# SamArgt/AudioSourceSep

Hardware: AMD Instinct MI355X
Metric: Glow fwd+logdet passes/sec on 64×64×1 mel tiles (K=32,L=3), 1→8 MI355X (higher is better)
Workload: dtype f16x3

## Files before the change

### audiosourcesep_amd/_lib.py

```python
import ctypes
import os

_HERE = os.path.dirname(os.path.abspath(__file__))
LIB_PATH = os.environ.get("GLOWK_LIB") or os.path.join(_HERE, "libglowk.so")


class GlowkLibraryMissing(RuntimeError):
    pass


class GlowkError(RuntimeError):
    pass


class GlowkRangeError(GlowkError):
    """GLOWK_ERR_RANGE: a call in a split arithmetic (f16x3 / f16x2) left the fp16 range; its outputs are not usable."""


class GlowkConfigStruct(ctypes.Structure):
    _fields_ = [
        ("H", ctypes.c_int32), ("W", ctypes.c_int32), ("C", ctypes.c_int32),
        ("L", ctypes.c_int32), ("K", ctypes.c_int32), ("F", ctypes.c_int32),
        ("learntop", ctypes.c_int32), ("use_logit", ctypes.c_int32),
        ("minval", ctypes.c_float), ("maxval", ctypes.c_float), ("alpha", ctypes.c_float),
        ("bn_eps", ctypes.c_float),
    ]


class GlowkProfile(ctypes.Structure):
    _fields_ = [("net_ms", ctypes.c_double * 4), ("net_launches", ctypes.c_int64 * 4)]


STEP_TENSOR_IDS = {
    "actnorm/log_scale": 0, "actnorm/shift": 1,
    "inv1x1/P": 2, "inv1x1/sign_S": 3, "inv1x1/L": 4, "inv1x1/log_S": 5, "inv1x1/U": 6,
    "nn/conv1/kernel": 7, "nn/conv1/bias": 8,
    "nn/bn1/gamma": 9, "nn/bn1/beta": 10, "nn/bn1/mean": 11, "nn/bn1/var": 12,
    "nn/conv2/kernel": 13, "nn/conv2/bias": 14,
    "nn/bn2/gamma": 15, "nn/bn2/beta": 16, "nn/bn2/mean": 17, "nn/bn2/var": 18,
    "nn/conv3/kernel": 19, "nn/conv3/bias": 20,
    "inv1x1/P_inv": 21,
}
PRIOR_TENSOR_IDS = {"prior/loc": 100, "prior/log_scale": 101}
PREC_F32, PREC_F16X3, PREC_F16X2 = 0, 1, 2
OK, ERR, ERR_RANGE = 0, 1, 2
RANGE_IGNORE, RANGE_ERROR, RANGE_FALLBACK = 0, 1, 2
MIX_DB, MIX_MEAN = 0, 1

_vp, _i, _fp = ctypes.c_void_p, ctypes.c_int, ctypes.POINTER(ctypes.c_float)

SYMBOLS = {
    "glowk_version": (_i, []),
    "glowk_last_error": (ctypes.c_char_p, []),
    "glowk_reload_env": (None, []),
    "glowk_create": (_i, [ctypes.POINTER(GlowkConfigStruct), _i, ctypes.POINTER(_vp)]),
    "glowk_destroy": (_i, [_vp]),
    "glowk_tensor_size": (ctypes.c_size_t, [_vp, _i, _i]),
    "glowk_set_tensor": (_i, [_vp, _i, _i, _i, _fp, ctypes.c_size_t]),
    "glowk_get_tensor": (_i, [_vp, _i, _i, _i, _fp, ctypes.c_size_t]),
    "glowk_finalize_weights": (_i, [_vp]),
    "glowk_actnorm_data_init": (_i, [_vp, _vp, _i, _i, _i, _vp]),
    "glowk_set_precision": (_i, [_vp, _i]),
    "glowk_get_precision": (_i, [_vp]),
    "glowk_set_range_policy": (_i, [_vp, _i]),
    "glowk_get_range_policy": (_i, [_vp]),
    "glowk_range_status": (_i, [_vp, ctypes.POINTER(_i), ctypes.POINTER(ctypes.c_int64), _vp]),
    "glowk_range_probe_begin": (_i, [_vp]),
    "glowk_range_probe_end": (_i, [_vp, ctypes.POINTER(ctypes.c_float), ctypes.POINTER(ctypes.c_float), _vp]),
    "glowk_workspace_bytes": (ctypes.c_size_t, [_vp, _i, _i]),
    "glowk_reserve": (_i, [_vp, _i, _i]),
    "glowk_max_tiles": (_i, [_vp]),
    "glowk_forward": (_i, [_vp, _vp, _i, _vp, _vp, _vp]),
    "glowk_inverse": (_i, [_vp, _vp, _i, _vp, _vp]),
    "glowk_log_prob": (_i, [_vp, _vp, _i, _vp, _vp, _vp]),
    "glowk_log_prob_sum": (_i, [_vp, _vp, _i, _vp, _vp, _vp, _i, _vp]),
    "glowk_sum_f64": (_i, [_vp, ctypes.c_size_t, _vp, _i, ctypes.c_double, _vp]),
    "glowk_log_prob_grad": (_i, [_vp, _vp, _i, _vp, _vp, _vp]),
    "glowk_sample": (_i, [_vp, _vp, _i, _vp, _vp]),
    "glowk_prior_log_prob": (_i, [_vp, _vp, _i, _vp, _vp]),
    "glowk_fused_steps": (ctypes.c_int64, [_vp]),
    "glowk_kernel_families": (_i, [_vp, ctypes.POINTER(ctypes.c_int64)]),
    "glowk_profile_begin": (_i, [_vp]),
    "glowk_profile_end": (_i, [_vp, ctypes.POINTER(GlowkProfile)]),
    "glowk_squeeze": (_i, [_vp, _i, _i, _i, _i, _vp, _vp]),
    "glowk_unsqueeze": (_i, [_vp, _i, _i, _i, _i, _vp, _vp]),
    "glowk_preprocess_forward": (_i, [_vp, _vp, _i, _vp, _vp, _vp]),
    "glowk_preprocess_inverse": (_i, [_vp, _vp, _i, _vp, _vp]),
    "glowk_step_forward": (_i, [_vp, _i, _i, _vp, _i, _vp, _vp, _vp]),
    "glowk_step_inverse": (_i, [_vp, _i, _i, _vp, _i, _vp, _vp]),
    "glowk_coupling_net": (_i, [_vp, _i, _i, _vp, _i, _vp, _vp, _vp]),
    "glowk_param_vector_size": (ctypes.c_size_t, [_vp]),
    "glowk_param_offset": (_i, [_vp, _i, _i, _i, ctypes.POINTER(ctypes.c_size_t), ctypes.POINTER(ctypes.c_size_t)]),
    "glowk_param_grad": (_i, [_vp, _vp, _i, ctypes.c_float, _vp, _vp, _vp]),
    "glowk_apply_gradients": (_i, [_vp, _vp, _i, ctypes.c_float, _vp]),
    "glowk_crc32c": (ctypes.c_uint32, [_vp, ctypes.c_size_t]),
    "glowk_basis_update": (_i, [_vp, _vp, _vp, _vp, _vp, ctypes.c_size_t, ctypes.c_float, ctypes.c_float, _vp, _vp,
                                ctypes.c_uint64, ctypes.c_uint64, ctypes.c_uint64, _vp, _vp]),
    "glowk_basis_mix": (_i, [_vp, _vp, _vp, ctypes.c_size_t, _vp]),
    "glowk_basis_update_n": (_i, [_vp, _vp, _vp, _i, _vp, ctypes.c_size_t, _i, ctypes.c_float, ctypes.c_float,
                                  ctypes.c_uint64, ctypes.c_uint64, ctypes.c_uint64, _vp, _vp]),
    "glowk_basis_mix_n": (_i, [_vp, _i, _vp, ctypes.c_size_t, _i, _vp]),
    "glowk_random_source": (_i, [_vp, ctypes.c_size_t, ctypes.c_uint64, ctypes.c_uint64, _i, _i, _i, ctypes.c_uint64, _vp]),
    "glowk_random": (_i, [_vp, ctypes.c_size_t, ctypes.c_uint64, ctypes.c_uint64, _i, _i, ctypes.c_uint64, _vp]),
    "glowk_add_noise": (_i, [_vp, _vp, ctypes.c_size_t, ctypes.c_float, ctypes.c_uint64, ctypes.c_uint64, _i, ctypes.c_uint64, _vp]),
    "glowk_mel_filterbank": (_i, [_fp]),
    "glowk_mel_frontend": (_i, [_vp, _i, _i, ctypes.c_float, _vp, _vp, _vp]),
    "glowk_mel_to_power": (_i, [_vp, _i, _i, _i, _vp, _vp]),
    "glowk_masked_istft": (_i, [_vp, _i, _vp, _i, _i, _i, _vp, _vp]),
    "glowk_griffinlim": (_i, [_vp, _vp, _i, _i, _i, ctypes.c_float, _vp, _vp]),
    "glowk_resample_length": (ctypes.c_int64, [ctypes.c_int64, _i, _i]),
    "glowk_resample_filter": (_i, [ctypes.POINTER(ctypes.c_double)]),
    "glowk_resample": (_i, [_vp, _i, ctypes.c_int64, _i, _i, _vp, _vp]),
    "glowk_bss_xcorr":(_i, [_vp, _i, ctypes.c_int64, _vp, _i, ctypes.c_int64, _vp, _i, _i, _vp, _vp]),
    "glowk_bss_solve": (_i, [_vp, _i, _i, _i, _i, _i, _vp, _i, _vp, _vp, _vp]),
    "glowk_bss_project": (_i, [_vp, ctypes.c_int64, _i, _i, _i, _vp, _i, ctypes.c_int64, _vp, _i, _vp, _i, _vp, _vp]),
    "glowk_sp_stft": (_i, [_vp, _i, ctypes.c_int64, _vp, _vp]),
    "glowk_sp_istft": (_i, [_vp, _i, _i, ctypes.c_int64, _vp, _vp]),
    "glowk_oracle_mask": (_i, [_vp, _i, _i, _i, _i, ctypes.c_double, ctypes.c_double, _vp, _vp]),
    "glowk_mwf": (_i, [_vp, _i, _i, _vp]),
    "glowk_oracle_mel": (_i, [_vp, _vp, _i, ctypes.c_int64, _i, _i, ctypes.c_double, _vp, _vp]),
    "glowk_mwf_em": (_i, [_vp, _vp, _i, _i, _i, _i, _vp, _vp, _vp]),
    "glowk_mel_frames": (_i, [_vp, _i, ctypes.c_int64, _vp, _vp, _vp]),
    "glowk_tile_cut": (_i, [_vp, _i, _i, _i, _i, ctypes.c_float, _vp, _vp]),
    "glowk_tile_stitch": (_i, [_vp, _i, _i, _i, _i, _i, _vp, _vp]),
}

_lib = None


def load():
    global _lib
    if _lib is not None:
        return _lib
    if not os.path.exists(LIB_PATH):
        raise GlowkLibraryMissing(
            "HIP library %s not found: build it first (python -c 'import __graft_entry__ as g; g.build()'). "
            "There is no CPU fallback for the compute path." % LIB_PATH)
    import torch
    lib = ctypes.CDLL(LIB_PATH)
    for name, (res, args) in SYMBOLS.items():
        fn = getattr(lib, name)
        fn.restype = res
        fn.argtypes = args
    _lib = lib
    return lib


def check(rc):
    if rc != 0:
        msg = load().glowk_last_error()
        raise (GlowkRangeError if rc == ERR_RANGE else GlowkError)(msg.decode() if msg else "glowk error %d" % rc)
```

### audiosourcesep_amd/csrc/glowk.hip

```cpp
#include "glowk_engine.h"
#include "glowk_light.h"

namespace glowk_eng {
thread_local std::string g_err;
}
using namespace glowk_eng;

namespace glowk_eng {

}

namespace glowk_detail {
int num_cus() {
  static int n = 0;
  if (n == 0) {
    int dev = 0; hipDeviceProp_t prop;
    if (hipGetDevice(&dev) == hipSuccess && hipGetDeviceProperties(&prop, dev) == hipSuccess) n = prop.multiProcessorCount;
    if (n <= 0) n = 256;
  }
  return n;
}
void launch_fail(const std::string& m) { fail(m); }
static EnvSwitches read_env() {
  auto on = [](const char* n) { return getenv(n) != nullptr; };
  return EnvSwitches{on("GLOWK_BWD_LIGHT_4"), on("GLOWK_NO_FUSE"), on("GLOWK_WGRAD_PLAIN"), on("GLOWK_CO_OFF"), on("GLOWK_CO_RING3"), on("GLOWK_Q_OFF"), on("GLOWK_CO_TRAIN_OFF"),
                     on("GLOWK_TRAIN_RECOMPUTE"), on("GLOWK_TRAIN_PERSTEP"), on("GLOWK_NO_PRESUM"), on("GLOWK_PG_JOIN")};
}
static EnvSwitches g_env = read_env();
const EnvSwitches& env() { return g_env; }
void reload_env() { g_env = read_env(); }
#define GLOWK_EXTERN_NET(CI_, NF_) extern template NetLaunch launch_net_t<CI_, NF_>(const NetArgs&, NetCall, hipStream_t, bool);
GLOWK_NET_SHAPES(GLOWK_EXTERN_NET)
#undef GLOWK_EXTERN_NET
}

namespace glowk_eng {
using glowk_detail::num_cus;
using glowk_detail::launch_net_t;

NetCall net_call(const glowk_handle* h, int dir, bool store, bool split) {
  if (h->precision == GLOWK_PREC_F32 || !split) return NetCall{dir, NET_EXACT, store};
  return NetCall{dir, h->precision == GLOWK_PREC_F16X2 && dir == NET_FWD && !store ? NET_SPLIT2 : NET_SPLIT3, store};
}

int* flagp(const glowk_handle* h) { return h->precision == GLOWK_PREC_F32 ? nullptr : h->d_flag; }

float bwd_norm_target(float xlim_b) {
  if (!(xlim_b >= 0.125f)) return 0.0f;
  int e = 0;
  std::frexp(xlim_b * 0.5f, &e);
  return std::ldexp(1.0f, std::min(e - 1, 10));
}

NetLaunch launch_net_raw(int c, int F, const NetArgs& a, NetCall call, hipStream_t s, bool dry) {
#define NETCASE(CI_, NF_) if (c == 2 * CI_ && F == 32 * NF_) return launch_net_t<CI_, NF_>(a, call, s, dry);
  GLOWK_NET_SHAPES(NETCASE)
#undef NETCASE
  return glowk_detail::net_failed("unsupported (channels, n_filters) combination: c=" + std::to_string(c) + " F=" + std::to_string(F));
}

int launch_net(glowk_handle* h, int level, int c, int F, const NetArgs& a, hipStream_t s, NetCall call, NetLaunch* out = nullptr) {
  if (h->profiling) {
    while (h->ev_pool.size() < h->ev_used + 2) {
      OwnedEvent e;
      HIPCHK(event_create(e, hipEventDefault));
      h->ev_pool.push_back(std::move(e));
    }
    HIPCHK(hipEventRecord(h->ev_pool[h->ev_used], s));
  }
  const NetLaunch r = launch_net_raw(c, F, a, call, s);
  if (!r.failed) {
    ++h->family_launches[r.family];
    if (r.co) ++h->family_launches[FAM_CO];
    if (r.q) ++h->family_launches[FAM_Q];
  }
  if (h->profiling) {
    HIPCHK(hipEventRecord(h->ev_pool[h->ev_used + 1], s));
    h->ev_used += 2;
    h->ev_level.push_back(level);
  }
  if (out) *out = r;
  return r.failed ? 1 : 0;
}


int launch_bwd_light(int c, const BwdArgs& a, int N, hipStream_t s) {
  const bool wide = c >= 8 && (a.Q + 15) / 16 <= 8 * num_cus() && !glowk_detail::env().bwd_light_4;
  auto al16 = [](const void* p) { return (reinterpret_cast<uintptr_t>(p) & 15) == 0; };
  const bool one = (a.Q + 255) / 256 >= 2 * num_cus() && al16(a.ghalf_in) && al16(a.v) && al16(a.osave) && al16(a.g_o) && al16(a.ghalf_out) &&
                   al16(a.gu_out) && al16(a.gv_out) && !glowk_detail::env().bwd_light_4;
  if (one) { CDISPATCH(c, hipLaunchKernelGGL((k_bwd_light<CC, 1>), dim3((a.Q + 255) / 256), dim3(256), 0, s, a)); }
  else if (wide) { CDISPATCH(c, hipLaunchKernelGGL((k_bwd_light<CC, 16>), dim3((a.Q + 15) / 16), dim3(256), 0, s, a)); }
  else { CDISPATCH(c, hipLaunchKernelGGL((k_bwd_light<CC, 4>), dim3((a.Q + 63) / 64), dim3(256), 0, s, a)); }
  LAUNCHCHK("k_bwd_light");
  return 0;
}

struct FlatLd { double* slot; int stride, base; };

#define PDISPATCH(c, CALL)                                                                     \
  switch (c) {                                                                                 \
    case 8: { constexpr int CC = 8; CALL; } break;                                             \
    case 16: { constexpr int CC = 16; CALL; } break;                                           \
    default: return fail("pre-summed P at channel count " + std::to_string(c));                \
  }

int launch_couple(int c, const CoupleArgs& a, int N, hipStream_t s, const FlatLd* fl = nullptr, bool* flat_used = nullptr) {
  const int hw = a.h * a.w;
  if (N < 2 * num_cus() && hw % 64 == 0 && (!a.logdet || (fl && fl->slot))) {
    CoupleArgs b = a;
    b.logdet = nullptr;
    double* slots = a.logdet ? fl->slot : (double*)nullptr;
    const bool wide = c >= 8 && (a.Q + 15) / 16 <= 8 * num_cus();
    if (a.presum) {
      if (wide) { PDISPATCH(c, hipLaunchKernelGGL((k_couple_flat<CC, 16, true>), dim3((a.Q + 15) / 16), dim3(256), 0, s, b, slots, fl ? fl->stride : 0, fl ? fl->base : 0)); }
      else { PDISPATCH(c, hipLaunchKernelGGL((k_couple_flat<CC, 4, true>), dim3((a.Q + 63) / 64), dim3(256), 0, s, b, slots, fl ? fl->stride : 0, fl ? fl->base : 0)); }
    }
    else if (wide) { CDISPATCH(c, hipLaunchKernelGGL((k_couple_flat<CC, 16>), dim3((a.Q + 15) / 16), dim3(256), 0, s, b, slots, fl ? fl->stride : 0, fl ? fl->base : 0)); }
    else { CDISPATCH(c, hipLaunchKernelGGL((k_couple_flat<CC, 4>), dim3((a.Q + 63) / 64), dim3(256), 0, s, b, slots, fl ? fl->stride : 0, fl ? fl->base : 0)); }
    LAUNCHCHK("k_couple_flat");
    if (flat_used && a.logdet) *flat_used = true;
    return 0;
  }
  if (N >= 2 * num_cus()) {
    if (a.presum) { PDISPATCH(c, hipLaunchKernelGGL((k_couple<CC, false, true>), dim3(N), dim3(256), 0, s, a)); }
    else { CDISPATCH(c, hipLaunchKernelGGL((k_couple<CC, false>), dim3(N), dim3(256), 0, s, a)); }
  } else {
    const int threads = hw >= 256 ? 1024 : hw > 64 ? 512 : 256;
    if (a.presum) { PDISPATCH(c, hipLaunchKernelGGL((k_couple<CC, true, true>), dim3(N), dim3(threads), 0, s, a)); }
    else { CDISPATCH(c, hipLaunchKernelGGL((k_couple<CC, true>), dim3(N), dim3(threads), 0, s, a)); }
  }
  LAUNCHCHK("k_couple");
  return 0;
}

bool fuse_geometry_ok(int h, int w, int pxw = 256) {
  const int hw = h * w;
  if (w < 4 || w > FUSE_EW || (w & (w - 1)) || pxw % w) return false;
  if (hw % pxw == 0) return true;
  return hw >= 32 && hw < pxw && (hw & (hw - 1)) == 0;
}

int net_and_couple(glowk_handle* h, int lvl, int c, int F, NetArgs na, CoupleArgs ca, int N, hipStream_t s, NetCall call, const FlatLd* fl = nullptr,
                   bool* flat_used = nullptr) {
  const bool no_fuse = glowk_detail::env().no_fuse;
  const bool fusable = call.arith != NET_EXACT && call.dir != NET_BWD && !call.store;
  const int hw = ca.h * ca.w;
  if (!no_fuse && c == 4 && fusable && na.RSp && ca.vin && !ca.log_s_out && ca.out && na.in_stride == 4 &&
      ca.out_stride % 4 == 0 && ca.out_off % 4 == 0 && fuse_geometry_ok(ca.h, ca.w) && na.P == h->bufP) {
    const size_t pxw = (na.co && fuse_geometry_ok(ca.h, ca.w, CO_PX)) ? CO_PX : 256;
    if (pxw == 256) na.co = 0;
    const size_t wgs = ((size_t)ca.Q + pxw - 1) / pxw;
    const size_t edge_floats = (wgs * 4 * FUSE_EW * 4 + 3) & ~(size_t)3;
    const size_t nld = wgs * (pxw / 32);
    if ((edge_floats + 2 * nld + 4) <= 4 * h->pstride) {
      na.fuse = 1;
      na.fz_b3 = ca.b3; na.fz_A = ca.A; na.fz_b = ca.b; na.fz_out = ca.out; na.fz_out_stride = ca.out_stride; na.fz_out_off = ca.out_off;
      na.fz_inverse = ca.inverse;
      na.fz_osave = ca.o_save;
      na.fz_edge = h->bufP;
      na.fz_ldpart = ca.logdet ? reinterpret_cast<double*>(h->bufP + edge_floats) : nullptr;
    }
  }
  NetLaunch r;
  if (int rc = launch_net(h, lvl, c, F, na, s, call, &r)) return rc;
  if (!r.fused_px) {
    ca.P = na.P; ca.np = r.np; ca.pstride = na.pstride; ca.presum = r.presum ? 1 : 0;
    return launch_couple(c, ca, N, s, fl, flat_used);
  }
  ++h->fused_steps;
  const int pxw = r.fused_px;
  if (hw > pxw || ca.logdet) {
    EdgeArgs ea;
    ea.vin = ca.vin; ea.edge = na.fz_edge; ea.ldpart = na.fz_ldpart; ea.A = ca.A; ea.b = ca.b; ea.out = ca.out; ea.out_stride = ca.out_stride;
    ea.out_off = ca.out_off; ea.inverse = ca.inverse; ea.logdet = ca.logdet; ea.osave = ca.o_save; ea.h = ca.h; ea.w = ca.w; ea.flag = ca.flag; ea.pxw = pxw;
    hipLaunchKernelGGL(k_couple_edge, dim3(N), dim3(256), 0, s, ea);
    LAUNCHCHK("k_couple_edge");
  }
  return 0;
}

PreArgs pre_args(const glowk_config& cfg) {
  PreArgs p;
  p.minval = cfg.minval; p.maxval = cfg.maxval; p.alpha = cfg.alpha; p.use_logit = cfg.use_logit;
  return p;
}

struct WsSizes {
  size_t act, P, ld;
  size_t slots;
  size_t total() const { return 3 * act + P + ld + slots; }
};
int ld_slots_per_sample(const glowk_handle* h) {
  int n = 0;
  for (const Level& lv : h->levels) n += h->cfg.K * ((lv.h * lv.w + 15) / 16);
  return n;
}
WsSizes ws_sizes(const glowk_handle* h, size_t N) {
  const size_t E = (size_t)h->cfg.H * h->cfg.W * h->cfg.C;
  return WsSizes{N * E * 4, 4 * 9 * N * E * 4, N * 8, std::min(N, (size_t)2 * num_cus()) * ld_slots_per_sample(h) * 8};
}
size_t mask_blocks(const Level& lv, size_t Q) {
  const size_t b256 = ((Q + 255) / 256) * 8;
  if (lv.c == 32) return ((Q + 127) / 128) * 8;
  const size_t Qh = (size_t)256 * (size_t)(num_cus() / 8);
  return std::max(b256, ((std::min(Q, Qh) + 127) / 128) * 8);
}

struct SaveSizes {
  size_t v, p, m;
  int np;
  size_t gz, c;
  size_t total() const { return v * 4 + (size_t)np * p * 4 + m * 2 + gz + c; }
};
SaveSizes save_sizes(const glowk_handle* h, size_t N, std::vector<size_t>* offV = nullptr, std::vector<size_t>* offP = nullptr,
                     std::vector<size_t>* offM = nullptr) {
  const int K = h->cfg.K, L = h->cfg.L, NF = h->cfg.F / 32;
  SaveSizes S{0, 0, 0, 1, 0, 0};
  if (offV) { offV->assign((size_t)L * K, 0); offP->assign((size_t)L * K, 0); offM->assign((size_t)L * K, 0); }
  for (int lvl = 0; lvl < L; ++lvl) {
    const Level& lv = h->levels[lvl];
    const size_t Q = N * lv.h * lv.w;
    const size_t blocks = mask_blocks(lv, Q);
    for (int j = 0; j < K; ++j) {
      const size_t sidx = (size_t)lvl * K + j;
      if (offV) { (*offV)[sidx] = S.v; (*offP)[sidx] = S.p; (*offM)[sidx] = S.m; }
      S.v += Q * lv.c;
      S.p += Q * (lv.c / 2);
      S.m += 2 * blocks * NF * 64;
    }
  }
  const size_t E = (size_t)h->cfg.H * h->cfg.W * h->cfg.C;
  S.gz = N * E * 4;
  S.c = N * E * 4;
  return S;
}

int ensure_flag(glowk_handle* h) {
  if (h->d_flag) return 0;
  DeviceMem<int> d_flag;
  PinnedMem<int> h_flag;
  HIPCHK(dev_alloc(d_flag, 16));
  HIPCHK(hipMemset(d_flag, 0, 16));
  HIPCHK(pinned_alloc(h_flag, 16));
  h_flag[0] = 0;
  h->d_flag = std::move(d_flag);
  h->h_flag = std::move(h_flag);
  return 0;
}

int ensure_ws(glowk_handle* h, int N) {
  if (int rc = ensure_flag(h)) return rc;
  if (N <= h->wsN) return 0;
  HIPCHK(hipDeviceSynchronize());
  h->bufA.reset(); h->bufB.reset(); h->bufP.reset(); h->bufZ.reset(); h->bufLd.reset(); h->bufLdSlot.reset(); h->wsN = 0;
  const WsSizes W = ws_sizes(h, (size_t)N);
  HIPCHK(dev_alloc(h->bufA, W.act));
  HIPCHK(dev_alloc(h->bufB, W.act));
  h->pstride = W.P / 16;
  HIPCHK(dev_alloc(h->bufP, W.P));
  HIPCHK(dev_alloc(h->bufZ, W.act));
  HIPCHK(dev_alloc(h->bufLd, W.ld));
  HIPCHK(dev_alloc(h->bufLdSlot, W.slots));
  h->wsN = N;
  return 0;
}

int ensure_c(glowk_handle* h, int N) {
  if ((size_t)N <= h->cN) return 0;
  HIPCHK(hipDeviceSynchronize());
  h->bufC.reset(); h->cN = 0;
  HIPCHK(dev_alloc(h->bufC, (size_t)N * h->cfg.H * h->cfg.W * h->cfg.C * 4));
  h->cN = (size_t)N;
  return 0;
}

int max_tiles(const glowk_handle* h) {
  const long long E = (long long)h->cfg.H * h->cfg.W * h->cfg.C;
  const long long m = (1LL << 28) / E;
  return m < 1 ? 1 : (int)m;
}


int check_batch(const glowk_handle* h, int N) {
  if (N <= 0) return fail("batch size must be positive");
  if (N > max_tiles(h)) return fail("batch of " + std::to_string(N) + " tiles exceeds glowk_max_tiles() = " + std::to_string(max_tiles(h)) +
                                    " (32-bit indices within one call): split the batch");
  return 0;
}

int check_ready(glowk_handle* h, int N) {
  if (!h) return fail("null handle");
  if (h->finalized && h->split_stale && h->precision != GLOWK_PREC_F32)
    if (int rc = glowk_finalize_weights(h)) return rc;
  if (!h->finalized) return fail("glowk_finalize_weights has not been called");
  if (int rc = check_batch(h, N)) return rc;
  return ensure_ws(h, N);
}

NetArgs net_args(glowk_handle* h, const Level& lv, const StepDev& sd, const float* vin, int in_stride, int in_off, int N) {
  NetArgs a;
  a.vin = vin; a.in_stride = in_stride; a.in_off = in_off;
  a.Q = N * lv.h * lv.w; a.h = lv.h; a.w = lv.w;
  a.K1p = sd.K1p; a.ep = sd.ep; a.R0p = sd.R0p; a.mask1 = nullptr; a.mask2 = nullptr; a.P = h->bufP;
  a.RHp = sd.RHp; a.RSp = sd.RSp; a.fam16 = (sd.RSp && sd.RSBp) ? 1 : 0; a.eph = sd.epH; a.pstride = h->pstride; a.max_np = 4; a.sc1 = sd.sc1; a.sc2 = sd.sc2; a.sc3 = sd.sc3;
  a.flag = flagp(h); a.xlim = sd.xlim_f; a.st1 = nullptr; a.st2 = nullptr;
  a.bnorm = 1.0f;
  a.fuse = 0; a.co = glowk_detail::env().co_off ? 0 : 1; a.fz_osave = nullptr; a.fz_b3 = nullptr; a.fz_A = nullptr; a.fz_b = nullptr; a.fz_out = nullptr; a.fz_out_stride = 0; a.fz_out_off = 0; a.fz_inverse = 0;
  a.fz_edge = nullptr; a.fz_ldpart = nullptr;
  a.pw = (!glowk_detail::env().no_presum && (lv.c == 8 || lv.c == 16) && lv.w >= 4 && lv.w <= 16 && (lv.w & (lv.w - 1)) == 0) ? lv.w : 0;
  a.pad = 0;
  a.xmax_out = h->d_probe ? h->d_probe + ((&lv - h->levels.data()) * h->cfg.K + (&sd - lv.dev.data())) : nullptr;
  return a;
}

int ensure_save(glowk_handle* h, int N) {
  if (int rc = ensure_c(h, N)) return rc;
  if (N <= h->saveN) return 0;
  const int Na = std::max(N, h->saveN);
  HIPCHK(hipDeviceSynchronize());
  h->saveV.reset(); h->saveP.reset(); h->saveM.reset(); h->bufGz.reset(); h->saveN = 0;
  SaveSizes S = save_sizes(h, (size_t)Na, &h->offV, &h->offP, &h->offM);
  HIPCHK(dev_alloc(h->saveV, S.v * 4));
  HIPCHK(dev_alloc(h->saveP, S.p * 4));
  HIPCHK(dev_alloc(h->saveM, S.m * 2));
  HIPCHK(dev_alloc(h->bufGz, S.gz));
  h->saveN = Na;
  return 0;
}

int run_forward(glowk_handle* h, const float* x, int N, float* z_dst, hipStream_t s, bool save, bool keep_hidden) {
  const glowk_config& cfg = h->cfg;
  const int K = cfg.K, L = cfg.L, NF = cfg.F / 32;
  float* cur = save ? h->saveV + h->offV[0] : h->bufA;
  float* oth = h->bufB;
  const int nslots = ld_slots_per_sample(h);
  const NetCall call = net_call(h, save ? NET_FWD_SAVE : NET_FWD, keep_hidden);
  const bool flat_ok = N < 2 * num_cus() && h->bufLdSlot;
  bool flat_used = false;
  int slot_base = 0;
  if (flat_ok) HIPCHK(hipMemsetAsync(h->bufLdSlot, 0, (size_t)N * nslots * 8, s));
  {
    const Level& lv = h->levels[0];
    const StepDev& first = lv.dev[K - 1];
    CDISPATCH(lv.c, hipLaunchKernelGGL((k_in<CC>), dim3(N), dim3(256), 0, s, x, cfg.H, cfg.W, pre_args(cfg), 1,
                                       first.Afwd, first.bfwd, cur, h->bufLd, h->ld_const + h->ld_pre_const));
    LAUNCHCHK("k_in");
  }
  for (int lvl = 0; lvl < L; ++lvl) {
    const Level& lv = h->levels[lvl];
    const size_t Q = (size_t)N * lv.h * lv.w;
    const size_t blocks = mask_blocks(lv, Q);
    for (int k = K - 1; k >= 0; --k) {
      const StepDev& sd = lv.dev[k];
      const size_t sidx = (size_t)lvl * K + (K - 1 - k);
      NetArgs na = net_args(h, lv, sd, cur, lv.c, lv.c / 2, N);
      if (save) {
        na.mask1 = h->saveM + h->offM[sidx];
        na.mask2 = na.mask1 + blocks * NF * 64;
      }
      if (keep_hidden) {
        na.st1 = h->trKeep + h->trKeepOff[sidx] * (size_t)N;
        na.st2 = na.st1 + (size_t)cfg.F * Q;
      }
      CoupleArgs ca;
      ca.presum = 0;
      ca.vin = cur; ca.b3 = sd.b3; ca.logdet = h->bufLd; ca.log_s_out = nullptr; ca.t_out = nullptr;
      ca.o_save = save ? h->saveP + h->offP[sidx] : nullptr;
      ca.Q = (int)Q; ca.h = lv.h; ca.w = lv.w; ca.inverse = 0; ca.flag = flagp(h);
      float* next = save && k > 0 ? h->saveV + h->offV[sidx + 1] : oth;
      if (k > 0) {
        ca.A = lv.dev[k - 1].Afwd; ca.b = lv.dev[k - 1].bfwd;
        ca.out = next; ca.out_stride = lv.c; ca.out_off = 0;
      } else if (lvl < L - 1) {
        ca.A = nullptr; ca.b = nullptr; ca.out = oth; ca.out_stride = lv.c; ca.out_off = 0;
      } else {
        ca.A = nullptr; ca.b = nullptr; ca.out = z_dst; ca.out_stride = h->Cl; ca.out_off = lv.z_off;
      }
      const FlatLd fl{flat_ok ? h->bufLdSlot : nullptr, nslots, slot_base};
      slot_base += (lv.h * lv.w + 15) / 16;
      if (int rc = net_and_couple(h, lvl, lv.c, cfg.F, na, ca, N, s, call, &fl, &flat_used)) return rc;
      if (k > 0) {
        if (save) cur = next; else std::swap(cur, oth);
      } else if (lvl < L - 1) {
        float* nv = save ? h->saveV + h->offV[sidx + 1] : cur;
        const StepDev& nfirst = h->levels[lvl + 1].dev[K - 1];
        CDISPATCH(lv.c, hipLaunchKernelGGL((k_split<CC>), dim3(N), dim3(256), 0, s, (const float*)oth, lv.h, lv.w, z_dst, h->Hl * h->Wl, h->Cl,
                                           lv.z_off, lv.Cz, nfirst.Afwd, nfirst.bfwd, nv));
        LAUNCHCHK("k_split");
        cur = nv;
        if (!save) oth = (cur == h->bufA) ? h->bufB : h->bufA;
      }
    }
  }
  if (flat_used) {
    hipLaunchKernelGGL(k_ld_fold, dim3(N), dim3(64), 0, s, h->bufLd, (const double*)h->bufLdSlot, nslots);
    LAUNCHCHK("k_ld_fold");
  }
  return 0;
}

int run_backward(glowk_handle* h, const float* x, const float* z, int N, float* dx, hipStream_t s, TrainCtx* tc) {
  const glowk_config& cfg = h->cfg;
  const int K = cfg.K, L = cfg.L, NF = cfg.F / 32;
  const int E = h->Hl * h->Wl * h->Cl;
  {
    const size_t total = (size_t)N * E;
    hipLaunchKernelGGL(k_prior_grad, dim3((unsigned)((total + 255) / 256)), dim3(256), 0, s, z, total, E, h->d_loc, h->d_log_scale, h->bufGz);
    LAUNCHCHK("k_prior_grad");
  }
  float* gh_a = h->bufA;
  float* gh_b = h->bufB;
  float* g_o = h->bufC;
  float* Pg = h->bufP;
  float* gu = h->bufZ;
  const float* gy_src = nullptr;
  for (int lvl = L - 1; lvl >= 0; --lvl) {
    const Level& lv = h->levels[lvl];
    const int Q = N * lv.h * lv.w;
    const size_t blocks = mask_blocks(lv, (size_t)Q);
    int npg = 1;
    const float bfac = (tc && tc->split && !h->tr_bfac.empty()) ? h->tr_bfac[lvl] : 1.0f;
    const bool level_batch = tc && h->trNB == K && K > 1;
    const size_t go_slot = level_batch ? (size_t)Q * lv.c : 0, m_slot = level_batch ? (size_t)cfg.F * Q : 0;
    const ptrdiff_t v_bs = K > 1 ? (ptrdiff_t)h->offV[(size_t)lvl * K] - (ptrdiff_t)h->offV[(size_t)lvl * K + 1] : 0;
    for (int k = 0; k < K; ++k) {
      const StepDev& sd = lv.dev[k];
      const size_t sidx = (size_t)lvl * K + (K - 1 - k);
      BwdArgs ba;
      ba.Q = Q; ba.h = lv.h; ba.w = lv.w; ba.flag = flagp(h);
      ba.go_scale = bfac; ba.pg_scale = 1.0f / bfac; ba.gmax = (tc && h->tr_gmax) ? h->tr_gmax + 16 * lvl : nullptr;
      ba.v = h->saveV + h->offV[sidx]; ba.osave = h->saveP + h->offP[sidx];
      float* go_k = tc ? h->trGo + (size_t)k * go_slot : g_o;
      ba.g_o = go_k; ba.ghalf_out = gh_b; ba.gu_out = nullptr;
      if (k == 0) {
        ba.ghalf_in = nullptr; ba.Pg = nullptr; ba.npg = 1; ba.pgstride = 0; ba.A = nullptr;
        if (lvl == L - 1) { ba.gv_direct = h->bufGz; ba.gvd_stride = h->Cl; ba.gvd_off = lv.z_off; }
        else              { ba.gv_direct = gy_src;   ba.gvd_stride = lv.c;  ba.gvd_off = 0; }
      } else {
        ba.ghalf_in = gh_a; ba.Pg = Pg; ba.npg = npg; ba.pgstride = h->pstride; ba.gv_direct = nullptr; ba.gvd_stride = 0; ba.gvd_off = 0;
        ba.A = lv.dev[k - 1].Afwd;
      }
      ba.gv_out = (tc && k > 0) ? h->trGv + (size_t)(k - 1) * go_slot : nullptr;
      if (int rc = launch_bwd_light(lv.c, ba, N, s)) return rc;
      if (tc && k > 0 && !level_batch)
        if (int rc = train_affine_sums(h, lvl, k - 1, 1, h->saveV + h->offV[sidx + 1], 0, h->trGv, 0, N, s)) return rc;
      std::swap(gh_a, gh_b);
      NetArgs na = net_args(h, lv, sd, go_k, lv.c, 0, N);
      na.K1p = sd.K3bp; na.R0p = sd.RBp; na.P = Pg;
      na.mask1 = h->saveM + h->offM[sidx];
      na.mask2 = na.mask1 + blocks * NF * 64;
      const NetCall call = net_call(h, NET_BWD, tc != nullptr, sd.RHBp || sd.RSBp);
      if (call.arith != NET_EXACT) {
        na.RHp = sd.RHBp; na.RSp = sd.RSBp; na.eph = nullptr; na.sc1 = sd.scb1; na.sc2 = sd.scb2; na.sc3 = sd.scb3; na.xlim = sd.xlim_b;
        na.bnorm = tc ? 1.0f : bwd_norm_target(sd.xlim_b);
        if (na.bnorm == 0.0f) {
          na.bnorm = 1.0f;
          if (na.flag) HIPCHK(hipMemsetAsync(na.flag, 1, sizeof(int), s));
        }
      }
      if (na.xmax_out) na.xmax_out += (size_t)cfg.L * cfg.K;
      if (tc) { na.st1 = h->trM2 + (size_t)k * m_slot; na.st2 = h->trM1 + (size_t)k * m_slot; }
      NetLaunch r;
      if (int rc = launch_net(h, lvl, lv.c, cfg.F, na, s, call, &r)) return rc;
      npg = r.np;
      if (tc && !level_batch) {
        const float* R1 = h->trR1;
        if (h->trKeep && N <= h->trKeepN) R1 = h->trKeep + h->trKeepOff[sidx] * (size_t)N;
        else {
          NetArgs nf = net_args(h, lv, sd, h->saveV + h->offV[sidx], lv.c, lv.c / 2, N);
          nf.P = h->bufP + 2 * h->pstride; nf.st1 = h->trR1; nf.st2 = h->trR1 + (size_t)cfg.F * Q;
          if (launch_net_raw(lv.c, cfg.F, nf, net_call(h, NET_FWD, true), s).failed) return 1;
        }
        if (int rc = train_network_grads(h, tc, lvl, k, 1, h->saveV + h->offV[sidx], 0, go_k, 0, R1, 0, h->trM1, h->trM2, 0, N, s, bfac)) return rc;
      }
    }
    {
      BwdArgs ba;
      ba.Q = Q; ba.h = lv.h; ba.w = lv.w; ba.flag = flagp(h);
      ba.go_scale = 1.0f; ba.pg_scale = 1.0f / bfac; ba.gmax = nullptr;
      ba.ghalf_in = gh_a; ba.Pg = Pg; ba.npg = npg; ba.pgstride = h->pstride; ba.gv_direct = nullptr; ba.gvd_stride = 0; ba.gvd_off = 0;
      ba.A = lv.dev[K - 1].Afwd;
      ba.v = nullptr; ba.osave = nullptr; ba.g_o = nullptr; ba.ghalf_out = nullptr; ba.gu_out = g_o;
      ba.gv_out = tc ? h->trGv + (size_t)(K - 1) * go_slot : nullptr;
      if (int rc = launch_bwd_light(lv.c, ba, N, s)) return rc;
      if (tc && !level_batch)
        if (int rc = train_affine_sums(h, lvl, K - 1, 1, h->saveV + h->offV[(size_t)lvl * K], 0, h->trGv, 0, N, s)) return rc;
    }
    if (level_batch) {
      const float* v0 = h->saveV + h->offV[(size_t)lvl * K + (K - 1)];
      const float* R10 = h->trKeep + h->trKeepOff[(size_t)lvl * K + (K - 1)] * (size_t)N;
      const ptrdiff_t r_bs = -(ptrdiff_t)(2 * (size_t)cfg.F * Q);
      if (int rc = train_affine_sums(h, lvl, 0, K, v0, v_bs, h->trGv, (ptrdiff_t)go_slot, N, s)) return rc;
      if (lvl == 0 && tc->sums_ready) { HIPCHK(hipEventRecord(tc->sums_ready, s)); tc->sums_ready = nullptr; }
      if (int rc = train_network_grads(h, tc, lvl, 0, K, v0, v_bs, h->trGo, (ptrdiff_t)go_slot, R10, r_bs, h->trM1, h->trM2, (ptrdiff_t)m_slot, N, s, bfac)) return rc;
    }
    if (lvl > 0) {
      const Level& pv = h->levels[lvl - 1];
      CDISPATCH(pv.c, hipLaunchKernelGGL((k_bwd_split<CC>), dim3(N), dim3(256), 0, s, (const float*)h->bufGz, h->Hl * h->Wl, h->Cl, pv.z_off,
                                         pv.Cz, (const float*)g_o, pv.h, pv.w, gu));
      LAUNCHCHK("k_bwd_split");
      gy_src = gu;
    } else {
      CDISPATCH(lv.c, hipLaunchKernelGGL((k_bwd_in<CC>), dim3(N), dim3(256), 0, s, (const float*)g_o, x, lv.h, lv.w, pre_args(cfg), dx));
      LAUNCHCHK("k_bwd_in");
    }
  }
  if (tc && tc->sums_ready) { HIPCHK(hipEventRecord(tc->sums_ready, s)); tc->sums_ready = nullptr; }
  return 0;
}

int run_inverse(glowk_handle* h, const float* z, int N, float* x, hipStream_t s) {
  const glowk_config& cfg = h->cfg;
  const int K = cfg.K, L = cfg.L;
  float* cur = h->bufA;
  float* oth = h->bufB;
  for (int lvl = L - 1; lvl >= 0; --lvl) {
    const Level& lv = h->levels[lvl];
    const float* unext = (lvl == L - 1) ? nullptr : cur;
    CDISPATCH(lv.c, hipLaunchKernelGGL((k_unsplit<CC>), dim3(N), dim3(256), 0, s, z, h->Hl * h->Wl, h->Cl, lv.z_off, lv.Cz, unext,
                                       lv.h, lv.w, oth));
    LAUNCHCHK("k_unsplit");
    std::swap(cur, oth);
    for (int k = 0; k < K; ++k) {
      const StepDev& sd = lv.dev[k];
      CoupleArgs ca;
      ca.vin = cur; ca.P = h->bufP; ca.np = 1; ca.pstride = h->pstride; ca.presum = 0; ca.b3 = sd.b3; ca.logdet = nullptr; ca.log_s_out = nullptr; ca.t_out = nullptr; ca.o_save = nullptr;
      ca.Q = N * lv.h * lv.w; ca.h = lv.h; ca.w = lv.w; ca.inverse = 1; ca.flag = flagp(h);
      ca.A = sd.Ainv; ca.b = sd.binv; ca.out = oth; ca.out_stride = lv.c; ca.out_off = 0;
      if (int rc = net_and_couple(h, lvl, lv.c, cfg.F, net_args(h, lv, sd, cur, lv.c, lv.c / 2, N), ca, N, s, net_call(h, NET_FWD))) return rc;
      std::swap(cur, oth);
    }
  }
  const Level& l0 = h->levels[0];
  CDISPATCH(l0.c, hipLaunchKernelGGL((k_out<CC>), dim3(N), dim3(256), 0, s, cur, l0.h, l0.w, pre_args(cfg), 1, x));
  LAUNCHCHK("k_out");
  return 0;
}

int launch_prior(glowk_handle* h, const float* z, int N, float* logp_dev, hipStream_t s) {
  hipLaunchKernelGGL(k_prior, dim3(N), dim3(256), 0, s, z, h->Hl * h->Wl * h->Cl, h->d_loc, h->d_log_scale, (const double*)h->bufLd, logp_dev, (float*)nullptr);
  LAUNCHCHK("k_prior");
  return 0;
}

int ptr_device(const void* p) {
  hipPointerAttribute_t a;
  int cur = 0;
  (void)hipGetDevice(&cur);
  if (hipPointerGetAttributes(&a, p) == hipSuccess && a.device >= 0) return a.device;
  (void)hipGetLastError();
  return cur;
}

template <class Run>
int guarded(glowk_handle* h, hipStream_t s, Run&& run) {
  if (int rc = run()) return rc;
  if (h->precision == GLOWK_PREC_F32 || h->range_policy == GLOWK_RANGE_IGNORE) return 0;
  HIPCHK(hipMemcpyAsync(h->h_flag, h->d_flag, sizeof(int), hipMemcpyDeviceToHost, s));
  HIPCHK(hipStreamSynchronize(s));
  if (!h->h_flag[0]) return 0;
  h->h_flag[0] = 0;
  HIPCHK(hipMemsetAsync(h->d_flag, 0, sizeof(int), s));
  if (h->range_policy == GLOWK_RANGE_ERROR) {
    g_err = "a hidden activation left the fp16 range of the split arithmetic (|a| >= 16 376) or the input is not finite: "
            "the outputs of this call are not usable -- use GLOWK_PREC_F32 or GLOWK_RANGE_FALLBACK";
    return GLOWK_ERR_RANGE;
  }
  const int prec = h->precision;
  h->precision = GLOWK_PREC_F32;
  ++h->range_fallbacks;
  const int rc = run();
  h->precision = prec;
  return rc;
}


}

extern "C" {

int glowk_version(void) { return GLOWK_VERSION; }
void glowk_reload_env(void) { glowk_detail::reload_env(); }
const char* glowk_last_error(void) { return g_err.c_str(); }

int glowk_create(const glowk_config* cfg, int device, glowk_handle** out) {
  if (!cfg || !out) return fail("null argument");
  if (cfg->L < 2 || cfg->L > 4) return fail("L should be 2, 3 or 4");
  const int s = 1 << cfg->L;
  if (cfg->H <= 0 || cfg->W <= 0 || cfg->C <= 0 || cfg->H % s || cfg->W % s) return fail("H and W must be positive multiples of 2^L");
  if (cfg->K <= 0) return fail("K must be positive");
  if (cfg->F != 128 && cfg->F != 256 && cfg->F != 384 && cfg->F != 512) return fail("n_filters must be 128, 256, 384 or 512 (the instantiated coupling-network widths)");
  glowk_handle* h = new glowk_handle();
  h->cfg = *cfg;
  h->device = device;
  h->Hl = cfg->H / s; h->Wl = cfg->W / s; h->Cl = cfg->C * s * s;
  int hh = cfg->H, ww = cfg->W, cc = cfg->C, off = 0, rem = h->Cl;
  for (int l = 0; l < cfg->L; ++l) {
    Level lv;
    hh /= 2; ww /= 2; cc *= 4;
    lv.h = hh; lv.w = ww; lv.c = cc;
    if (l < cfg->L - 1) {
      lv.z_width = rem / 2; lv.z_off = off; off += lv.z_width; rem -= lv.z_width;
      lv.Cz = (hh * ww * (cc / 2)) / (h->Hl * h->Wl);
    } else {
      lv.z_width = rem; lv.z_off = off; lv.Cz = 0;
    }
    for (int t = 0; t < GLOWK_NUM_STEP_TENSORS; ++t) {
      lv.host[t].resize(cfg->K);
      for (int k = 0; k < cfg->K; ++k) lv.host[t][k].assign(step_tensor_size(*cfg, lv, t), 0.0f);
    }
    lv.dev.resize(cfg->K);
    h->levels.push_back(std::move(lv));
    cc /= 2;
  }
  const size_t E = (size_t)h->Hl * h->Wl * h->Cl;
  h->prior_loc.assign(E, 0.0f);
  h->prior_log_scale.assign(E, 0.0f);
  *out = h;
  return 0;
}

int glowk_destroy(glowk_handle* h) {
  if (!h) return 0;
  DeviceGuard dg(h->device);
  (void)hipDeviceSynchronize();
  delete h;
  return 0;
}

size_t glowk_tensor_size(const glowk_handle* h, int level, int tensor_id) {
  if (!h) return 0;
  if (tensor_id == GLOWK_PRIOR_LOC || tensor_id == GLOWK_PRIOR_LOG_SCALE) return h->prior_loc.size();
  if (level < 0 || level >= (int)h->levels.size() || tensor_id < 0 || tensor_id >= GLOWK_NUM_STEP_TENSORS) return 0;
  return step_tensor_size(h->cfg, h->levels[level], tensor_id);
}

static std::vector<float>* locate(glowk_handle* h, int level, int step, int id) {
  if (id == GLOWK_PRIOR_LOC) return &h->prior_loc;
  if (id == GLOWK_PRIOR_LOG_SCALE) return &h->prior_log_scale;
  if (level < 0 || level >= (int)h->levels.size() || id < 0 || id >= GLOWK_NUM_STEP_TENSORS) return nullptr;
  if (step < 0 || step >= h->cfg.K) return nullptr;
  return &h->levels[level].host[id][step];
}

int glowk_set_tensor(glowk_handle* h, int level, int step, int tensor_id, const float* host, size_t n) {
  if (!h || !host) return fail("null argument");
  if (h->host_stale) { DeviceGuard dg(h->device); if (int rc = sync_host(h)) return rc; }
  h->tr_active = false;
  std::vector<float>* v = locate(h, level, step, tensor_id);
  if (!v) return fail("no such tensor");
  if (v->size() != n) return fail("tensor size mismatch: expected " + std::to_string(v->size()) + ", got " + std::to_string(n));
  std::memcpy(v->data(), host, n * sizeof(float));
  h->finalized = false;
  return 0;
}

int glowk_get_tensor(const glowk_handle* h, int level, int step, int tensor_id, float* host, size_t n) {
  if (!h || !host) return fail("null argument");
  if (h->host_stale) { DeviceGuard dg(h->device); if (int rc = sync_host(const_cast<glowk_handle*>(h))) return rc; }
  const std::vector<float>* v = locate(const_cast<glowk_handle*>(h), level, step, tensor_id);
  if (!v) return fail("no such tensor");
  if (v->size() != n) return fail("tensor size mismatch");
  std::memcpy(host, v->data(), n * sizeof(float));
  if (tensor_id == GLOWK_INV1X1_P_INV) {
    bool set = false;
    for (size_t i = 0; i < n; ++i) set |= host[i] != 0.0f;
    if (!set) {
      const int c = h->levels[level].c;
      const std::vector<float>& P = h->levels[level].host[GLOWK_INV1X1_P][step];
      Mat Pm(P.begin(), P.end()), Pi;
      if (invert(Pm, c, Pi))
        for (size_t i = 0; i < n; ++i) host[i] = (float)Pi[i];
    }
  }
  return 0;
}

int glowk_finalize_weights(glowk_handle* h) {
  if (!h) return fail("null handle");
  if (h->host_stale) { DeviceGuard dg0(h->device); if (int rc = sync_host(h)) return rc; }
  const glowk_config& cfg = h->cfg;
  for (const Level& lv : h->levels)
    if (lv.c != 4 && lv.c != 8 && lv.c != 16 && lv.c != 32)
      return fail("unsupported channel count " + std::to_string(lv.c) + " (this build: 4, 8, 16, 32)");
  size_t total = 0;
  for (const Level& lv : h->levels) total += step_layout(lv.c, cfg.F).total * cfg.K;
  const size_t E = h->prior_loc.size();
  const size_t prior_off = total;
  total += 2 * pad4(E);
  std::vector<float> stage(total, 0.0f);
  std::vector<PackJob> jobs;
  std::vector<size_t> offs;
  {
    size_t o = 0;
    for (size_t l = 0; l < h->levels.size(); ++l)
// ... 76 lines not shown
  ca.out = cur; ca.out_stride = lv.c; ca.out_off = 0;
  ca.logdet = nullptr; ca.log_s_out = nullptr; ca.t_out = nullptr;
  ca.Q = Q; ca.h = lv.h; ca.w = lv.w; ca.inverse = 0; ca.flag = nullptr;
  return launch_couple(lv.c, ca, Nl, s);
}

int refresh_step_affine(glowk_handle* h, int lvl, int k, hipStream_t s) {
  Level& lv = h->levels[lvl];
  const StepLayout SL = step_layout(lv.c, h->cfg.F);
  std::vector<float> tmp(SL.total - SL.Afwd + SL.Afwd, 0.0f);
  std::string err;
  double ldc = 0;
  if (!pack_affine(h->cfg, lv, k, tmp.data(), &ldc, &err)) return fail(err);
  h->ld_step[(size_t)lvl * h->cfg.K + k] = ldc;
  HIPCHK(hipMemcpyAsync(h->arena + lv.dev[k].arena_off + SL.Afwd, tmp.data() + SL.Afwd, (SL.total - SL.Afwd) * 4, hipMemcpyHostToDevice, s));
  HIPCHK(hipStreamSynchronize(s));
  return 0;
}
}

int glowk_actnorm_data_init(glowk_handle* h, const float* x_dev, int N, int runtime_order, int raw_minibatch_quirk, void* stream) {
  if (!h) return fail("null handle");
  DeviceGuard dg(h->device);
  if (int rc = check_ready(h, N)) return rc;
  if (!x_dev) return fail("null tensor");
  hipStream_t s = (hipStream_t)stream;
  const glowk_config& cfg = h->cfg;
  const int K = cfg.K, L = cfg.L;
  const size_t E = (size_t)cfg.H * cfg.W * cfg.C;
  if (int rc = ensure_c(h, N)) return rc;
  if (h->host_stale) if (int rc = sync_host(h)) return rc;
  h->tr_active = false;
  if (!h->bufStat) HIPCHK(dev_alloc(h->bufStat, (size_t)(STAT_BLOCKS + 1) * 32 * 8));
  hipLaunchKernelGGL(k_pre_only, dim3(N), dim3(256), 0, s, x_dev, (int)E, pre_args(cfg), 0, h->bufZ, (float*)nullptr, 0.0);
  LAUNCHCHK("k_pre_only");
  PreArgs nopre = {0, 1, 0, 0};
  float* blk_in = h->bufC;
  float* cur = h->bufA;
  float* tmp = h->bufB;
  const bool quirk = raw_minibatch_quirk && L > 2;
  std::vector<double> part((size_t)STAT_BLOCKS * 32), mean(32), var(32);
  for (int lvl = 0; lvl < L; ++lvl) {
    Level& lv = h->levels[lvl];
    int Nl = N;
    if (lvl == 0) {
      CDISPATCH(lv.c, hipLaunchKernelGGL((k_in<CC>), dim3(N), dim3(256), 0, s, (const float*)h->bufZ, cfg.H, cfg.W, nopre, 0,
                                         (const float*)nullptr, (const float*)nullptr, blk_in, (double*)nullptr, 0.0));
      LAUNCHCHK("k_in");
    } else if (quirk) {
      Nl = (int)((size_t)N * E / ((size_t)lv.h * lv.w * lv.c));
      CDISPATCH(lv.c, hipLaunchKernelGGL((k_in<CC>), dim3(Nl), dim3(256), 0, s, (const float*)h->bufZ, 2 * lv.h, 2 * lv.w, nopre, 0,
                                         (const float*)nullptr, (const float*)nullptr, blk_in, (double*)nullptr, 0.0));
      LAUNCHCHK("k_in");
    } else {
      const Level& pv = h->levels[lvl - 1];
      CDISPATCH(pv.c, hipLaunchKernelGGL((k_split<CC>), dim3(N), dim3(256), 0, s, (const float*)cur, pv.h, pv.w, (float*)nullptr, 0, 0, 0, 1,
                                         (const float*)nullptr, (const float*)nullptr, blk_in));
      LAUNCHCHK("k_split");
    }
    const int Q = Nl * lv.h * lv.w;
    HIPCHK(hipMemcpyAsync(cur, blk_in, (size_t)Q * lv.c * 4, hipMemcpyDeviceToDevice, s));
    for (int idx = 0; idx < K; ++idx) {
      const int k = runtime_order ? K - 1 - idx : idx;
      double* d_part = h->bufStat;
      double* d_mean = h->bufStat + (size_t)STAT_BLOCKS * 32;
      for (int pass = 0; pass < 2; ++pass) {
        CDISPATCH(lv.c, hipLaunchKernelGGL((k_chan_stats<CC>), dim3(STAT_BLOCKS), dim3(256), 0, s, (const float*)cur, Q,
                                           pass ? (const double*)d_mean : (const double*)nullptr, d_part));
        LAUNCHCHK("k_chan_stats");
        HIPCHK(hipMemcpyAsync(part.data(), d_part, (size_t)STAT_BLOCKS * lv.c * 8, hipMemcpyDeviceToHost, s));
        HIPCHK(hipStreamSynchronize(s));
        for (int c = 0; c < lv.c; ++c) {
          double t = 0;
          for (int b = 0; b < STAT_BLOCKS; ++b) t += part[(size_t)b * lv.c + c];
          (pass ? var : mean)[c] = t / Q;
        }
        if (!pass) HIPCHK(hipMemcpyAsync(d_mean, mean.data(), lv.c * 8, hipMemcpyHostToDevice, s));
      }
      for (int c = 0; c < lv.c; ++c) {
        const double sd_ = (double)((float)std::sqrt(var[c]) + 1e-8f);
        lv.host[GLOWK_ACTNORM_LOG_SCALE][k][c] = (float)std::log(1.0 / sd_);
        lv.host[GLOWK_ACTNORM_SHIFT][k][c] = (float)(-mean[c] / sd_);
      }
      if (int rc = refresh_step_affine(h, lvl, k, s)) return rc;
      if (int rc = run_step_inplace(h, lvl, k, cur, tmp, Nl, s)) return rc;
    }
    if (lvl < L - 1 && !quirk && !runtime_order) {
      HIPCHK(hipMemcpyAsync(cur, blk_in, (size_t)Q * lv.c * 4, hipMemcpyDeviceToDevice, s));
      for (int k = K - 1; k >= 0; --k)
        if (int rc = run_step_inplace(h, lvl, k, cur, tmp, Nl, s)) return rc;
    }
  }
  h->ld_const = 0.0;
  for (double v : h->ld_step) h->ld_const += v;
  HIPCHK(hipStreamSynchronize(s));
  return 0;
}

int glowk_set_precision(glowk_handle* h, int precision) {
  if (!h) return fail("null handle");
  if (precision != GLOWK_PREC_F32 && precision != GLOWK_PREC_F16X3 && precision != GLOWK_PREC_F16X2) return fail("unknown precision mode");
  h->precision = precision;
  return 0;
}

int glowk_get_precision(const glowk_handle* h) { return h ? h->precision : -1; }

int glowk_set_range_policy(glowk_handle* h, int policy) {
  if (!h) return fail("null handle");
  if (policy != GLOWK_RANGE_IGNORE && policy != GLOWK_RANGE_ERROR && policy != GLOWK_RANGE_FALLBACK) return fail("unknown range policy");
  h->range_policy = policy;
  return 0;
}

int glowk_get_range_policy(const glowk_handle* h) { return h ? h->range_policy : -1; }

int glowk_range_status(glowk_handle* h, int* tripped, int64_t* fallbacks, void* stream) {
  if (!h) return fail("null handle");
  DeviceGuard dg(h->device);
  if (fallbacks) *fallbacks = h->range_fallbacks;
  if (tripped) {
    *tripped = 0;
    if (h->d_flag) {
      hipStream_t s = (hipStream_t)stream;
      HIPCHK(hipMemcpyAsync(h->h_flag, h->d_flag, sizeof(int), hipMemcpyDeviceToHost, s));
      HIPCHK(hipStreamSynchronize(s));
      if (h->h_flag[0]) {
        *tripped = 1;
        h->h_flag[0] = 0;
        HIPCHK(hipMemsetAsync(h->d_flag, 0, sizeof(int), s));
      }
    }
  }
  return 0;
}

int glowk_range_probe_begin(glowk_handle* h) {
  if (!h) return fail("null handle");
  DeviceGuard dg(h->device);
  const size_t n = (size_t)2 * h->cfg.L * h->cfg.K;
  if (!h->d_probe) HIPCHK(dev_alloc(h->d_probe, n * sizeof(unsigned)));
  HIPCHK(hipMemset(h->d_probe, 0, n * sizeof(unsigned)));
  return 0;
}

int glowk_range_probe_end(glowk_handle* h, float* fwd_ratio, float* bwd_ratio, void* stream) {
  if (!h) return fail("null handle");
  if (!h->d_probe) return fail("glowk_range_probe_end without glowk_range_probe_begin");
  DeviceGuard dg(h->device);
  const int LK = h->cfg.L * h->cfg.K;
  std::vector<float> v((size_t)2 * LK);
  HIPCHK(hipStreamSynchronize((hipStream_t)stream));
  HIPCHK(hipMemcpy(v.data(), h->d_probe, v.size() * sizeof(float), hipMemcpyDeviceToHost));
  h->d_probe.reset();
  float rf = 0.f, rb = 0.f;
  for (int l = 0; l < h->cfg.L; ++l)
    for (int k = 0; k < h->cfg.K; ++k) {
      const StepDev& sd = h->levels[l].dev[k];
      const int i = l * h->cfg.K + k;
      if (sd.xlim_f > 0.f) rf = std::max(rf, v[i] / sd.xlim_f);
      if (sd.xlim_b > 0.f && v[LK + i] > 0.f) rb = std::max(rb, 0.125f / sd.xlim_b);
    }
  if (fwd_ratio) *fwd_ratio = rf;
  if (bwd_ratio) *bwd_ratio = rb;
  return 0;
}

size_t glowk_workspace_bytes(const glowk_handle* h, int N, int with_grad) {
  if (!h || N <= 0) return 0;
  size_t b = ws_sizes(h, (size_t)N).total() + 16 ;
  if (with_grad) b += save_sizes(h, (size_t)N).total();
  return b;
}

int glowk_max_tiles(const glowk_handle* h) { return h ? max_tiles(h) : 0; }

int glowk_reserve(glowk_handle* h, int N, int with_grad) {
  if (!h) return fail("null handle");
  DeviceGuard dg(h->device);
  if (int rc = check_batch(h, N)) return rc;
  if (int rc = ensure_ws(h, N)) return rc;
  if (with_grad) {
    if (!h->finalized) return fail("glowk_finalize_weights must run before reserving the gradient path (its size depends on the launch policy)");
    return ensure_save(h, N);
  }
  return 0;
}

int glowk_forward(glowk_handle* h, const float* x_dev, int N, float* z_dev, float* logdet_dev, void* stream) {
  if (!h) return fail("null handle");
  DeviceGuard dg(h->device);
  if (int rc = check_ready(h, N)) return rc;
  if (!x_dev || !z_dev) return fail("null tensor");
  hipStream_t s = (hipStream_t)stream;
  return guarded(h, s, [&]() -> int {
    if (int rc = run_forward(h, x_dev, N, z_dev, s)) return rc;
    if (logdet_dev) {
      hipLaunchKernelGGL(k_prior, dim3(N), dim3(256), 0, s, (const float*)nullptr, 0, (const float*)nullptr, (const float*)nullptr,
                         (const double*)h->bufLd, (float*)nullptr, logdet_dev);
      LAUNCHCHK("k_prior(logdet)");
    }
    return 0;
  });
}

int glowk_inverse(glowk_handle* h, const float* z_dev, int N, float* x_dev, void* stream) {
  if (!h) return fail("null handle");
  DeviceGuard dg(h->device);
  if (int rc = check_ready(h, N)) return rc;
  if (!x_dev || !z_dev) return fail("null tensor");
  hipStream_t s = (hipStream_t)stream;
  return guarded(h, s, [&]() -> int { return run_inverse(h, z_dev, N, x_dev, s); });
}

int glowk_log_prob(glowk_handle* h, const float* x_dev, int N, float* logp_dev, float* z_dev, void* stream) {
  if (!h) return fail("null handle");
  DeviceGuard dg(h->device);
  if (int rc = check_ready(h, N)) return rc;
  if (!x_dev || !logp_dev) return fail("null tensor");
  hipStream_t s = (hipStream_t)stream;
  float* z = z_dev ? z_dev : h->bufZ;
  return guarded(h, s, [&]() -> int {
    if (int rc = run_forward(h, x_dev, N, z, s)) return rc;
    hipLaunchKernelGGL(k_prior, dim3(N), dim3(256), 0, s, (const float*)z, h->Hl * h->Wl * h->Cl, h->d_loc, h->d_log_scale,
                       (const double*)h->bufLd, logp_dev, (float*)nullptr);
    LAUNCHCHK("k_prior");
    return 0;
  });
}

int glowk_log_prob_sum(glowk_handle* h, const float* x_dev, int N, float* logp_dev, float* z_dev, double* sum_dev, int accumulate, void* stream) {
  if (!h) return fail("null handle");
  DeviceGuard dg(h->device);
  if (int rc = check_ready(h, N)) return rc;
  if (!x_dev || !logp_dev || !sum_dev) return fail("null tensor");
  hipStream_t s = (hipStream_t)stream;
  float* z = z_dev ? z_dev : h->bufZ;
  const int rc = guarded(h, s, [&]() -> int {
    if (int rc = run_forward(h, x_dev, N, z, s)) return rc;
    hipLaunchKernelGGL(k_prior, dim3(N), dim3(256), 0, s, (const float*)z, h->Hl * h->Wl * h->Cl, h->d_loc, h->d_log_scale,
                       (const double*)h->bufLd, logp_dev, (float*)nullptr);
    LAUNCHCHK("k_prior");
    return 0;
  });
  if (rc) return rc;
  hipLaunchKernelGGL(k_sum_f64, dim3(1), dim3(1024), 0, s, (const float*)logp_dev, (size_t)N, sum_dev, accumulate, 1.0);
  LAUNCHCHK("k_sum_f64");
  return 0;
}

int glowk_sum_f64(const float* v_dev, size_t n, double* out_dev, int accumulate, double scale, void* stream) {
  if (!out_dev || (!v_dev && n)) return fail("null tensor");
  DeviceGuard dg(ptr_device(out_dev));
  hipLaunchKernelGGL(k_sum_f64, dim3(1), dim3(1024), 0, (hipStream_t)stream, v_dev, n, out_dev, accumulate, scale);
  LAUNCHCHK("k_sum_f64");
  return 0;
}

int glowk_log_prob_grad(glowk_handle* h, const float* x_dev, int N, float* logp_dev, float* dx_dev, void* stream) {
  if (!h) return fail("null handle");
  DeviceGuard dg(h->device);
  if (int rc = check_ready(h, N)) return rc;
  if (!x_dev || !logp_dev || !dx_dev) return fail("null tensor");
  if (int rc = ensure_save(h, N)) return rc;
  hipStream_t s = (hipStream_t)stream;
  float* z = h->bufGz;
  return guarded(h, s, [&]() -> int {
    if (int rc = run_forward(h, x_dev, N, z, s, true)) return rc;
    hipLaunchKernelGGL(k_prior, dim3(N), dim3(256), 0, s, (const float*)z, h->Hl * h->Wl * h->Cl, h->d_loc, h->d_log_scale,
                       (const double*)h->bufLd, logp_dev, (float*)nullptr);
    LAUNCHCHK("k_prior");
    return run_backward(h, x_dev, z, N, dx_dev, s);
  });
}

int glowk_sample(glowk_handle* h, const float* eps_dev, int N, float* x_dev, void* stream) {
  if (!h) return fail("null handle");
  DeviceGuard dg(h->device);
  if (int rc = check_ready(h, N)) return rc;
  if (!eps_dev || !x_dev) return fail("null tensor");
  hipStream_t s = (hipStream_t)stream;
  const int E = h->Hl * h->Wl * h->Cl;
  const size_t total = (size_t)N * E;
  return guarded(h, s, [&]() -> int {
    hipLaunchKernelGGL(k_prior_sample, dim3((unsigned)((total + 255) / 256)), dim3(256), 0, s, eps_dev, total, E, h->d_loc, h->d_log_scale,
                       h->bufZ);
    LAUNCHCHK("k_prior_sample");
    return run_inverse(h, h->bufZ, N, x_dev, s);
  });
}

int glowk_prior_log_prob(glowk_handle* h, const float* z_dev, int N, float* logp_dev, void* stream) {
  if (!h) return fail("null handle");
  DeviceGuard dg(h->device);
  if (int rc = check_ready(h, N)) return rc;
  if (!z_dev || !logp_dev) return fail("null tensor");
  hipLaunchKernelGGL(k_prior, dim3(N), dim3(256), 0, (hipStream_t)stream, z_dev, h->Hl * h->Wl * h->Cl, h->d_loc, h->d_log_scale,
                     (const double*)nullptr, logp_dev, (float*)nullptr);
  LAUNCHCHK("k_prior");
  return 0;
}

int64_t glowk_fused_steps(const glowk_handle* h) { return h ? h->fused_steps : -1; }

int glowk_kernel_families(const glowk_handle* h, int64_t* out7) {
  if (!h || !out7) return fail("null argument");
  for (int i = 0; i < FAM_COUNT; ++i) out7[i] = h->family_launches[i];
  return 0;
}

int glowk_profile_begin(glowk_handle* h) {
  if (!h) return fail("null handle");
  h->profiling = true;
  h->ev_used = 0;
  h->ev_level.clear();
  return 0;
}

int glowk_profile_end(glowk_handle* h, glowk_profile* out) {
  if (!h || !out) return fail("null argument");
  std::memset(out, 0, sizeof(*out));
  h->profiling = false;
  DeviceGuard dg(h->device);
  HIPCHK(hipDeviceSynchronize());
  for (size_t i = 0; i < h->ev_level.size(); ++i) {
    float ms = 0.0f;
    HIPCHK(hipEventElapsedTime(&ms, h->ev_pool[2 * i], h->ev_pool[2 * i + 1]));
    const int l = h->ev_level[i];
    if (l >= 0 && l < 4) { out->net_ms[l] += ms; out->net_launches[l] += 1; }
  }
  h->ev_used = 0;
  h->ev_level.clear();
  return 0;
}

int glowk_squeeze(const float* x_dev, int N, int H, int W, int C, float* y_dev, void* stream) {
  if (!x_dev || !y_dev) return fail("null tensor");
  if (N <= 0 || H <= 0 || W <= 0 || H % 2 || W % 2) return fail("squeeze needs even H and W");
  if ((long long)N * H * W * C > (1LL << 28)) return fail("squeeze: more than 2^28 elements in one call; split the batch");
  DeviceGuard dg(ptr_device(x_dev));
  PreArgs p = {0, 1, 0, 0};
  const int c = 4 * C;
  CDISPATCH(c, hipLaunchKernelGGL((k_in<CC>), dim3(N), dim3(256), 0, (hipStream_t)stream, x_dev, H, W, p, 0, (const float*)nullptr,
                                  (const float*)nullptr, y_dev, (double*)nullptr, 0.0));
  LAUNCHCHK("k_in(squeeze)");
  return 0;
}

int glowk_unsqueeze(const float* y_dev, int N, int hh, int ww, int c4, float* x_dev, void* stream) {
  if (!x_dev || !y_dev) return fail("null tensor");
  if (N <= 0 || hh <= 0 || ww <= 0 || c4 % 4) return fail("unsqueeze needs a channel count divisible by 4");
  if ((long long)N * hh * ww * c4 > (1LL << 28)) return fail("unsqueeze: more than 2^28 elements in one call; split the batch");
  DeviceGuard dg(ptr_device(y_dev));
  PreArgs p = {0, 1, 0, 0};
  CDISPATCH(c4, hipLaunchKernelGGL((k_out<CC>), dim3(N), dim3(256), 0, (hipStream_t)stream, y_dev, hh, ww, p, 0, x_dev));
  LAUNCHCHK("k_out(unsqueeze)");
  return 0;
}

int glowk_preprocess_forward(glowk_handle* h, const float* x_dev, int N, float* y_dev, float* logdet_dev, void* stream) {
  if (!h || !x_dev || !y_dev) return fail("null argument");
  DeviceGuard dg(h->device);
  if (int rc = check_batch(h, N)) return rc;
  const int E = h->cfg.H * h->cfg.W * h->cfg.C;
  double ldc = -(double)E * std::log((double)h->cfg.maxval - (double)h->cfg.minval);
  if (h->cfg.use_logit) ldc += (double)E * std::log(1.0 - 2.0 * (double)h->cfg.alpha);
  hipLaunchKernelGGL(k_pre_only, dim3(N), dim3(256), 0, (hipStream_t)stream, x_dev, E, pre_args(h->cfg), 0, y_dev, logdet_dev, ldc);
  LAUNCHCHK("k_pre_only");
  return 0;
}

int glowk_preprocess_inverse(glowk_handle* h, const float* y_dev, int N, float* x_dev, void* stream) {
  if (!h || !x_dev || !y_dev) return fail("null argument");
  DeviceGuard dg(h->device);
  if (int rc = check_batch(h, N)) return rc;
  const int E = h->cfg.H * h->cfg.W * h->cfg.C;
  hipLaunchKernelGGL(k_pre_only, dim3(N), dim3(256), 0, (hipStream_t)stream, y_dev, E, pre_args(h->cfg), 1, x_dev, (float*)nullptr, 0.0);
  LAUNCHCHK("k_pre_only");
  return 0;
}

int glowk_step_forward(glowk_handle* h, int level, int step, const float* u_dev, int N, float* y_dev, float* logdet_dev, void* stream) {
  if (!h) return fail("null handle");
  DeviceGuard dg(h->device);
  if (int rc = check_ready(h, N)) return rc;
  if (level < 0 || level >= h->cfg.L || step < 0 || step >= h->cfg.K) return fail("no such step");
  if (!u_dev || !y_dev) return fail("null tensor");
  hipStream_t s = (hipStream_t)stream;
  const Level& lv = h->levels[level];
  const StepDev& sd = lv.dev[step];
  const int Q = N * lv.h * lv.w;
  return guarded(h, s, [&]() -> int {
    CDISPATCH(lv.c, hipLaunchKernelGGL((k_affine<CC>), dim3((Q + 255) / 256), dim3(256), 0, s, u_dev, Q, sd.Afwd, sd.bfwd, h->bufA));
    LAUNCHCHK("k_affine");
    NetLaunch r;
    if (int rc = launch_net(h, level, lv.c, h->cfg.F, net_args(h, lv, sd, h->bufA, lv.c, lv.c / 2, N), s, net_call(h, NET_FWD), &r)) return rc;
    if (logdet_dev) {
      std::vector<double> init(N, h->ld_step[(size_t)level * h->cfg.K + step]);
      HIPCHK(hipMemcpyAsync(h->bufLd, init.data(), (size_t)N * 8, hipMemcpyHostToDevice, s));
      HIPCHK(hipStreamSynchronize(s));
    }
    CoupleArgs ca;
    ca.o_save = nullptr;
    ca.vin = h->bufA; ca.P = h->bufP; ca.np = r.np; ca.pstride = h->pstride; ca.presum = r.presum ? 1 : 0; ca.b3 = sd.b3; ca.A = nullptr; ca.b = nullptr;
    ca.out = y_dev; ca.out_stride = lv.c; ca.out_off = 0;
    ca.logdet = logdet_dev ? h->bufLd : nullptr; ca.log_s_out = nullptr; ca.t_out = nullptr;
    ca.Q = Q; ca.h = lv.h; ca.w = lv.w; ca.inverse = 0; ca.flag = flagp(h);
    if (int rc = launch_couple(lv.c, ca, N, s)) return rc;
    if (logdet_dev) {
      hipLaunchKernelGGL(k_prior, dim3(N), dim3(256), 0, s, (const float*)nullptr, 0, (const float*)nullptr, (const float*)nullptr,
                         (const double*)h->bufLd, (float*)nullptr, logdet_dev);
      LAUNCHCHK("k_prior(logdet)");
    }
    return 0;
  });
}

int glowk_step_inverse(glowk_handle* h, int level, int step, const float* y_dev, int N, float* u_dev, void* stream) {
  if (!h) return fail("null handle");
  DeviceGuard dg(h->device);
  if (int rc = check_ready(h, N)) return rc;
  if (level < 0 || level >= h->cfg.L || step < 0 || step >= h->cfg.K) return fail("no such step");
  if (!u_dev || !y_dev) return fail("null tensor");
  hipStream_t s = (hipStream_t)stream;
  const Level& lv = h->levels[level];
  const StepDev& sd = lv.dev[step];
  return guarded(h, s, [&]() -> int {
    NetLaunch r;
    if (int rc = launch_net(h, level, lv.c, h->cfg.F, net_args(h, lv, sd, y_dev, lv.c, lv.c / 2, N), s, net_call(h, NET_FWD), &r)) return rc;
    CoupleArgs ca;
    ca.o_save = nullptr;
    ca.vin = y_dev; ca.P = h->bufP; ca.np = r.np; ca.pstride = h->pstride; ca.presum = r.presum ? 1 : 0; ca.b3 = sd.b3; ca.A = sd.Ainv; ca.b = sd.binv;
    ca.out = u_dev; ca.out_stride = lv.c; ca.out_off = 0;
    ca.logdet = nullptr; ca.log_s_out = nullptr; ca.t_out = nullptr;
    ca.Q = N * lv.h * lv.w; ca.h = lv.h; ca.w = lv.w; ca.inverse = 1; ca.flag = flagp(h);
    return launch_couple(lv.c, ca, N, s);
  });
}

int glowk_coupling_net(glowk_handle* h, int level, int step, const float* xb_dev, int N, float* log_s_dev, float* t_dev, void* stream) {
  if (!h) return fail("null handle");
  DeviceGuard dg(h->device);
  if (int rc = check_ready(h, N)) return rc;
  if (level < 0 || level >= h->cfg.L || step < 0 || step >= h->cfg.K) return fail("no such step");
  if (!xb_dev || !log_s_dev || !t_dev) return fail("null tensor");
  hipStream_t s = (hipStream_t)stream;
  const Level& lv = h->levels[level];
  const StepDev& sd = lv.dev[step];
  return guarded(h, s, [&]() -> int {
    NetLaunch r;
    if (int rc = launch_net(h, level, lv.c, h->cfg.F, net_args(h, lv, sd, xb_dev, lv.c / 2, 0, N), s, net_call(h, NET_FWD), &r)) return rc;
    CoupleArgs ca;
    ca.o_save = nullptr;
    ca.vin = nullptr; ca.P = h->bufP; ca.np = r.np; ca.pstride = h->pstride; ca.presum = r.presum ? 1 : 0; ca.b3 = sd.b3; ca.A = nullptr; ca.b = nullptr;
    ca.out = nullptr; ca.out_stride = 0; ca.out_off = 0;
    ca.logdet = nullptr; ca.log_s_out = log_s_dev; ca.t_out = t_dev;
    ca.Q = N * lv.h * lv.w; ca.h = lv.h; ca.w = lv.w; ca.inverse = 0; ca.flag = flagp(h);
    return launch_couple(lv.c, ca, N, s);
  });
}


}
```

### audiosourcesep_amd/csrc/glowk_engine.h

```cpp
#pragma once
#include "../../include/glowk.h"
#include "glowk_kernels.h"
#include "glowk_pack.h"
#include "glowk_launch.h"

#include <algorithm>
#include <atomic>
#include <cmath>
#include <cstdio>
#include <cstdlib>
#include <cstring>
#include <sched.h>
#include <string>
#include <thread>
#include <vector>

namespace glowk_eng {

extern thread_local std::string g_err;

inline int fail(const std::string& m) {
  g_err = m;
  return GLOWK_ERR;
}

struct DeviceGuard {
  int prev = -1;
  bool changed = false;
  explicit DeviceGuard(int dev) {
    if (hipGetDevice(&prev) == hipSuccess && prev != dev) changed = hipSetDevice(dev) == hipSuccess;
  }
  ~DeviceGuard() {
    if (changed) (void)hipSetDevice(prev);
  }
  DeviceGuard(const DeviceGuard&) = delete;
  DeviceGuard& operator=(const DeviceGuard&) = delete;
};

#define HIPCHK(expr)                                                                           \
  do {                                                                                         \
    hipError_t e_ = (expr);                                                                    \
    if (e_ != hipSuccess) return glowk_eng::fail(std::string(#expr) + ": " + hipGetErrorString(e_));      \
  } while (0)

#define LAUNCHCHK(name)                                                                        \
  do {                                                                                         \
    hipError_t e_ = hipGetLastError();                                                         \
    if (e_ != hipSuccess) return glowk_eng::fail(std::string("launch ") + name + ": " + hipGetErrorString(e_)); \
  } while (0)

template <class T, class Release>
class Owner {
 public:
  Owner() = default;
  explicit Owner(Release r) : r_(r) {}
  Owner(Owner&& o) noexcept : p_(o.release()), r_(o.r_) {}
  Owner& operator=(Owner&& o) noexcept { reset(o.release()); r_ = o.r_; return *this; }
  ~Owner() { reset(); }
  operator T() const { return p_; }
  const Release& releaser() const { return r_; }
  T release() { T p = p_; p_ = nullptr; return p; }
  void reset(T p = nullptr) { if (p_) r_(p_); p_ = p; }
 private:
  T p_ = nullptr;
  Release r_{};
};
struct HipFree { void operator()(void* p) const { (void)hipFree(p); } };
struct HipHostFree { void operator()(void* p) const { (void)hipHostFree(p); } };
struct HipFreeAsync { hipStream_t s; void operator()(void* p) const { (void)hipFreeAsync(p, s); } };
struct HipStreamDestroy { void operator()(hipStream_t s) const { (void)hipStreamDestroy(s); } };
struct HipEventDestroy { void operator()(hipEvent_t e) const { (void)hipEventDestroy(e); } };
template <class T> using DeviceMem = Owner<T*, HipFree>;
template <class T> using PinnedMem = Owner<T*, HipHostFree>;
template <class T> using Scratch = Owner<T*, HipFreeAsync>;
using OwnedStream = Owner<hipStream_t, HipStreamDestroy>;
using OwnedEvent = Owner<hipEvent_t, HipEventDestroy>;

template <class T, class R, class Create>
hipError_t create_into(Owner<T, R>& o, Create create) {
  o.reset();
  T p = nullptr;
  const hipError_t e = create(&p);
  if (e == hipSuccess) o.reset(p);
  return e;
}
template <class T> hipError_t dev_alloc(DeviceMem<T>& o, size_t bytes) { return create_into(o, [&](T** p) { return hipMalloc(p, bytes); }); }
template <class T> hipError_t pinned_alloc(PinnedMem<T>& o, size_t bytes) { return create_into(o, [&](T** p) { return hipHostMalloc(p, bytes); }); }
template <class T> hipError_t scratch_alloc(Scratch<T>& o, size_t bytes) {
  return create_into(o, [&](T** p) { return hipMallocAsync(reinterpret_cast<void**>(p), bytes, o.releaser().s); });
}
inline hipError_t stream_create(OwnedStream& o) { return create_into(o, [](hipStream_t* s) { return hipStreamCreateWithFlags(s, hipStreamNonBlocking); }); }
inline hipError_t event_create(OwnedEvent& o, unsigned flags) { return create_into(o, [&](hipEvent_t* e) { return hipEventCreateWithFlags(e, flags); }); }

}
using glowk_eng::DeviceMem; using glowk_eng::PinnedMem; using glowk_eng::OwnedStream; using glowk_eng::OwnedEvent;

struct glowk_handle {
  glowk_config cfg;
  int device = 0;
  int precision = GLOWK_PREC_F32;
  int range_policy = GLOWK_RANGE_ERROR;
  int64_t range_fallbacks = 0;
  int64_t family_launches[FAM_COUNT] = {};
  int64_t fused_steps = 0;
  DeviceMem<int> d_flag;
  PinnedMem<int> h_flag;
  DeviceMem<unsigned> d_probe;
  std::vector<Level> levels;
  int Hl = 0, Wl = 0, Cl = 0;
  std::vector<float> prior_loc, prior_log_scale;
  bool finalized = false;
  double ld_const = 0.0;
  double ld_pre_const = 0.0;
  std::vector<double> ld_step;
  DeviceMem<float> arena;
  const float* d_loc = nullptr;
  const float* d_log_scale = nullptr;
  int wsN = 0;
  DeviceMem<float> bufA, bufB, bufP, bufZ, bufC;
  size_t pstride = 0;
  DeviceMem<double> bufLd;
  DeviceMem<double> bufLdSlot;
  DeviceMem<double> bufStat;
  int saveN = 0;
  size_t cN = 0;
  DeviceMem<float> saveV, saveP, bufGz;
  DeviceMem<unsigned short> saveM;
  std::vector<size_t> offV, offP, offM;
  bool tr_active = false;
  bool host_stale = false;
  bool split_stale = false;
  DeviceMem<float> tr_params, tr_m, tr_v;
  size_t tr_n = 0;
  long tr_t = 0;
  std::vector<size_t> tr_level_off;
  size_t tr_prior_off = 0;
  std::vector<DeviceMem<int>> tr_map;
  std::vector<size_t> tr_map_n;
  std::vector<DeviceMem<int>> tr_map16;
  std::vector<size_t> tr_map16_n;
  DeviceMem<float> tr16_src;
  DeviceMem<int> tr16_S;
  DeviceMem<float> tr16_scales;
  size_t tr16_src_max = 0;
  PinnedMem<float> tr_pinned;
  std::vector<size_t> tr_pin_off;
  std::vector<OwnedStream> tr_streams;
  std::vector<OwnedEvent> tr_events;
  std::vector<float> tr_bfac;
  DeviceMem<unsigned> tr_gmax;
  PinnedMem<float> h_gmax;
  OwnedStream tr_side;
  OwnedEvent tr_ev_sums, tr_ev_up;
  PinnedMem<double> h_sums;
  PinnedMem<float> h_up;
  int trN = 0;
  DeviceMem<float> trR1, trM1, trM2, trXcol, trGcol, trCpart, trC1, trC2, trC3, trGv, trGo;
  int trNB = 1;
  DeviceMem<double> trAffPart, trAffSum;
  DeviceMem<float> trKeep;
  std::vector<size_t> trKeepOff;
  int trKeepN = 0;
  bool profiling = false;
  std::vector<OwnedEvent> ev_pool;
  size_t ev_used = 0;
  std::vector<int> ev_level;
};

#define CDISPATCH(c, CALL)                                                                     \
  switch (c) {                                                                                 \
    case 4: { constexpr int CC = 4; CALL; } break;                                             \
    case 8: { constexpr int CC = 8; CALL; } break;                                             \
    case 16: { constexpr int CC = 16; CALL; } break;                                           \
    case 32: { constexpr int CC = 32; CALL; } break;                                           \
    default: return glowk_eng::fail("unsupported channel count " + std::to_string(c));         \
  }

namespace glowk_eng {

struct TrainCtx {
  float* grad;
  float scale;
  bool split;
  hipEvent_t sums_ready = nullptr;
};

int check_ready(glowk_handle* h, int N);
int ensure_save(glowk_handle* h, int N);
NetArgs net_args(glowk_handle* h, const Level& lv, const StepDev& sd, const float* vin, int in_stride, int in_off, int N);
NetCall net_call(const glowk_handle* h, int dir, bool store = false, bool split = true);
NetLaunch launch_net_raw(int c, int F, const NetArgs& a, NetCall call, hipStream_t s, bool dry = false);
int run_forward(glowk_handle* h, const float* x, int N, float* z_dst, hipStream_t s, bool save = false, bool keep_hidden = false);
int run_backward(glowk_handle* h, const float* x, const float* z, int N, float* dx, hipStream_t s, TrainCtx* tc = nullptr);
int launch_prior(glowk_handle* h, const float* z, int N, float* logp_dev, hipStream_t s);
int ptr_device(const void* p);

int sync_host(glowk_handle* h);
int train_network_grads(glowk_handle* h, TrainCtx* tc, int lvl, int k0, int nb, const float* v, ptrdiff_t v_bs, const float* g_o, ptrdiff_t go_bs,
                        const float* R1, ptrdiff_t r_bs, const float* M1, const float* M2, ptrdiff_t m_bs, int N, hipStream_t s, float bfac = 1.0f);
int train_affine_sums(glowk_handle* h, int lvl, int k0, int nb, const float* v, ptrdiff_t v_bs, const float* gv, ptrdiff_t gv_bs, int N, hipStream_t s);

}
```

### audiosourcesep_amd/csrc/glowk_kernels.h

```cpp
#pragma once
#include "glowk_act_scale.h"

#include <hip/hip_runtime.h>
#include <utility>
#include <stdint.h>

typedef float f32x16 __attribute__((ext_vector_type(16)));

#define GLOWK_GPTR(p) ((const __attribute__((address_space(1))) void*)(p))
#define GLOWK_LPTR(p) ((__attribute__((address_space(3))) void*)(p))

__device__ __forceinline__ int mfma_row(int r, int hh) { return (r & 3) + 8 * (r >> 2) + 4 * hh; }

struct NetArgs {
  const float* vin;
  int in_stride, in_off;
  int Q, h, w;
  const float* K1p;
  const float* ep;
  const float4* R0p;
  unsigned short* mask1;
  unsigned short* mask2;
  float* P;
  size_t pstride;
  int max_np;
  const float4* RHp;
  const float* eph;
  const float4* RSp;
  int fam16;
  float sc1, sc2, sc3;
  int* flag;
  float xlim;
  float bnorm;
  int fuse;
  int co;
  const float* fz_b3;
  const float* fz_A;
  const float* fz_b;
  float* fz_out;
  int fz_out_stride, fz_out_off, fz_inverse;
  float* fz_osave;
  float* fz_edge;
  double* fz_ldpart;
  unsigned* xmax_out;
  float* st1;
  float* st2;
  int pw;
  int pad;
};
static_assert(sizeof(NetArgs) == 264, "kernel argument size");

#define GLOWK_ST_MOD " nt"
__device__ __forceinline__ void st_tile_planar(float* blk_base, unsigned lane_byte, unsigned row_bytes, const f32x16& v) {
  const unsigned long long base = reinterpret_cast<unsigned long long>(blk_base);
  unsigned off = lane_byte;
#pragma unroll
  for (int r = 0; r < 16; ++r) {
    asm volatile("global_store_dword %0, %1, %2" GLOWK_ST_MOD ::"v"(off), "v"(v[r]), "s"(base) : "memory");
    off += ((r & 3) == 3 ? 5u : 1u) * row_bytes;
  }
}

template <int C>
__device__ __forceinline__ void affine_cc(const float* __restrict__ A, const float* __restrict__ b, const float (&x)[C], float (&y)[C]) {
#pragma unroll
  for (int co = 0; co < C; ++co) y[co] = b[co];
#pragma unroll
  for (int ci = 0; ci < C; ++ci)
#pragma unroll
    for (int co = 0; co < C; ++co) y[co] = fmaf(x[ci], A[ci * C + co], y[co]);
}

__device__ __forceinline__ void glds16(const float4* src_lane, float4* lds_wave_base) {
  __builtin_amdgcn_global_load_lds(GLOWK_GPTR(src_lane), GLOWK_LPTR(lds_wave_base), 16, 0, 0);
}

__device__ __forceinline__ float* uniform_fptr(float* p) {
  const unsigned long long b = reinterpret_cast<unsigned long long>(p);
  const unsigned lo = __builtin_amdgcn_readfirstlane((unsigned)b);
  const unsigned hi = __builtin_amdgcn_readfirstlane((unsigned)(b >> 32));
  return reinterpret_cast<float*>(((unsigned long long)hi << 32) | lo);
}
__device__ __forceinline__ const char* uniform_ptr(const void* p) {
  const unsigned long long b = reinterpret_cast<unsigned long long>(p);
  const unsigned lo = __builtin_amdgcn_readfirstlane((unsigned)b);
  const unsigned hi = __builtin_amdgcn_readfirstlane((unsigned)(b >> 32));
  return reinterpret_cast<const char*>(((unsigned long long)hi << 32) | lo);
}

template <int P>
__device__ __forceinline__ float4* ring_slot(float4* s0, float4* s1) { return P ? s1 : s0; }

template <int KIN, int NF>
struct Ring1 {
  static constexpr int KS1 = (9 * KIN) / 2;
  static constexpr int MAIN4 = NF * 256;
  static constexpr int K1PIECES_FULL = (KS1 * 256 + 1023) / 1024;
  static constexpr bool K1_IN_RING = (size_t)2 * (MAIN4 + K1PIECES_FULL * 64) * 16 + (size_t)6 * NF * 32 * 4 <= 160 * 1024;
  static constexpr int K1PIECES = K1_IN_RING ? K1PIECES_FULL : 0;
  static constexpr bool K1_IN_BUF = !K1_IN_RING && (size_t)2 * MAIN4 * 16 + (size_t)6 * NF * 32 * 4 + (size_t)K1PIECES_FULL * 1024 <= 160 * 1024;
  static constexpr int K1HALF_KS = KS1 / 2;
  static constexpr int K1HALF_PIECES = (K1HALF_KS * 256 + 1023) / 1024;
  static constexpr bool K1_IN_HALF = !K1_IN_RING && !K1_IN_BUF && KS1 % 2 == 0 && (K1HALF_KS * 256) % 1024 == 0 &&
                                     (size_t)2 * MAIN4 * 16 + (size_t)6 * NF * 32 * 4 + (size_t)K1HALF_PIECES * 1024 <= 160 * 1024;
  static constexpr int K1BUF4 = K1_IN_BUF ? K1PIECES_FULL * 64 : K1_IN_HALF ? K1HALF_PIECES * 64 : 1;
  static constexpr int SLOT4 = MAIN4 + K1PIECES * 64;
  static constexpr int PIECES = NF * 4 + K1PIECES;
  static constexpr size_t LDS_BYTES = (size_t)2 * SLOT4 * 16 + (size_t)6 * NF * 32 * 4 + ((K1_IN_BUF || K1_IN_HALF) ? (size_t)K1BUF4 * 16 : 0);
  static constexpr bool FITS = LDS_BYTES <= 160 * 1024;
};

template <int P0, int N>
__device__ __forceinline__ void stage_range(const float4* __restrict__ src, float4* dst, int wave, unsigned voff) {
  const char* gb = uniform_ptr(src);
#pragma unroll
  for (int i = 0; i < (N + 3) / 4; ++i) {
    int p = i * 4 + wave;
    p = P0 + (p < N ? p : N - 1);
    glds16(reinterpret_cast<const float4*>(gb + (size_t)p * 1024 + voff), dst + p * 64);
  }
}

enum { NET_FWD = 0, NET_FWD_SAVE = 1, NET_BWD = 2,
       NET_FWD2 = 3 };
constexpr int NET_STORE = 8;
constexpr int NET_FUSE = 16;
constexpr int NET_HALF = 32;
template <int MODE>
constexpr int net_dir = MODE & 7;

template <int N>
__device__ __forceinline__ unsigned pick_word(const unsigned (&w)[N], int j) {
  unsigned r = 0;
#pragma unroll
  for (int i = 0; i < N; ++i) r = (j == i) ? w[i] : r;
  return r;
}

template <int KIN, int NF, int P, int MODE, bool STORE>
__device__ __forceinline__ void net_step(const NetArgs& a, int fi, bool first, const float4* nsrc, float4* s0, float4* s1, float4* k1buf,
                                         const float* epl, const float (&xcol)[(9 * KIN) / 2], f32x16 (&acc2)[NF],
                                         const unsigned (&mk)[NF / 2], size_t wblk, int wave, unsigned voff, int lane, int hh, int q, bool qok, bool wok) {
  using G = Ring1<KIN, NF>;
  constexpr int KS1 = G::KS1;
  constexpr int F = NF * 32;
  f32x16 h1;
#pragma unroll
  for (int r = 0; r < 16; ++r) h1[r] = 0.0f;
  if constexpr (G::K1_IN_HALF) {
    constexpr int KH = G::K1HALF_KS;
    if (!first) {
      asm volatile("s_waitcnt vmcnt(0)" ::: "memory");
      __syncthreads();
    }
    const float* k1 = reinterpret_cast<const float*>(k1buf) + lane;
#pragma unroll
    for (int ks = 0; ks < KH; ++ks) h1 = __builtin_amdgcn_mfma_f32_32x32x2f32(k1[ks * 64], xcol[ks], h1, 0, 0, 0);
    __syncthreads();
    stage_range<0, G::K1HALF_PIECES>(reinterpret_cast<const float4*>(a.K1p + ((size_t)fi * KS1 + KH) * 64), k1buf, wave, voff);
    asm volatile("s_waitcnt vmcnt(0)" ::: "memory");
    __syncthreads();
#pragma unroll
    for (int ks = 0; ks < KH; ++ks) h1 = __builtin_amdgcn_mfma_f32_32x32x2f32(k1[ks * 64], xcol[KH + ks], h1, 0, 0, 0);
  } else {
    if (G::K1_IN_BUF && !first) {
      asm volatile("s_waitcnt vmcnt(0)" ::: "memory");
      __syncthreads();
    }
    const float* k1 = G::K1_IN_RING ? reinterpret_cast<const float*>(ring_slot<P ^ 1>(s0, s1) + G::MAIN4) + lane
                      : G::K1_IN_BUF ? reinterpret_cast<const float*>(k1buf) + lane
                                     : a.K1p + (size_t)fi * KS1 * 64 + lane;
#pragma unroll
    for (int ks = 0; ks < KS1; ++ks) h1 = __builtin_amdgcn_mfma_f32_32x32x2f32(k1[ks * 64], xcol[ks], h1, 0, 0, 0);
  }
  float* st_blk = STORE ? uniform_fptr(a.st1 + (size_t)fi * 32 * a.Q) : nullptr;
  const unsigned st_lane = STORE ? ((unsigned)(4 * hh) * (unsigned)a.Q + (unsigned)q) * 4u : 0u;
  const unsigned st_row = (unsigned)a.Q * 4u;
  if (MODE == NET_BWD) {
    const unsigned w = pick_word<NF / 2>(mk, fi >> 1) >> ((fi & 1) * 16);
#pragma unroll
    for (int r = 0; r < 16; ++r) h1[r] = ((w >> r) & 1u) ? h1[r] : 0.0f;
    if (STORE && qok) st_tile_planar(st_blk, st_lane, st_row, h1);
#pragma unroll
    for (int r = 0; r < 16; ++r) h1[r] *= epl[4 * F + fi * 32 + mfma_row(r, hh)];
  } else {
    unsigned bits = 0;
#pragma unroll
    for (int r = 0; r < 16; ++r) {
      const int f = fi * 32 + mfma_row(r, hh);
      const float pre = h1[r] + epl[f];
      if (MODE == NET_FWD_SAVE) bits |= (pre > 0.0f ? 1u : 0u) << r;
      h1[r] = fmaxf(pre, 0.0f);
    }
    if (STORE && qok) st_tile_planar(st_blk, st_lane, st_row, h1);
#pragma unroll
    for (int r = 0; r < 16; ++r) {
      const int f = fi * 32 + mfma_row(r, hh);
      h1[r] = fmaf(epl[F + f], h1[r], epl[2 * F + f]);
    }
    if (MODE == NET_FWD_SAVE) a.mask1[(wblk * NF + fi) * 64 + lane] = (unsigned short)bits;
  }
  {
    constexpr int NST = (STORE ? 16 : 0) + (MODE == NET_FWD_SAVE ? 1 : 0);
    if (!first || G::K1_IN_BUF) {
      if (NST && wok) asm volatile("s_waitcnt vmcnt(%0)" ::"n"(NST) : "memory");
      else asm volatile("s_waitcnt vmcnt(0)" ::: "memory");
    }
    __syncthreads();
  }
  stage_range<0, G::PIECES>(nsrc, ring_slot<P ^ 1>(s0, s1), wave, voff);
  if (G::K1_IN_BUF && fi + 1 < NF)
    stage_range<0, G::K1PIECES_FULL>(reinterpret_cast<const float4*>(a.K1p + (size_t)(fi + 1) * KS1 * 64), k1buf, wave, voff);
  if constexpr (G::K1_IN_HALF) {
    if (fi + 1 < NF) stage_range<0, G::K1HALF_PIECES>(reinterpret_cast<const float4*>(a.K1p + (size_t)(fi + 1) * KS1 * 64), k1buf, wave, voff);
  }
  const float4* buf = ring_slot<P>(s0, s1);
#pragma unroll
  for (int r = 0; r < 16; ++r) {
#pragma unroll
    for (int g = 0; g < NF / 4; ++g) {
      const float4 wv = buf[(r * (NF / 4) + g) * 64 + lane];
      acc2[4 * g + 0] = __builtin_amdgcn_mfma_f32_32x32x2f32(wv.x, h1[r], acc2[4 * g + 0], 0, 0, 0);
      acc2[4 * g + 1] = __builtin_amdgcn_mfma_f32_32x32x2f32(wv.y, h1[r], acc2[4 * g + 1], 0, 0, 0);
      acc2[4 * g + 2] = __builtin_amdgcn_mfma_f32_32x32x2f32(wv.z, h1[r], acc2[4 * g + 2], 0, 0, 0);
      acc2[4 * g + 3] = __builtin_amdgcn_mfma_f32_32x32x2f32(wv.w, h1[r], acc2[4 * g + 3], 0, 0, 0);
    }
  }
}

template <int KIN, int MOUT, int NF, int MODE, bool STORE = false>
__global__ __launch_bounds__(256, 1) void k_net_f32(NetArgs a) {
  using G = Ring1<KIN, NF>;
  constexpr int KS1 = G::KS1;
  constexpr int NMT = (MOUT + 31) / 32;
  constexpr int F = NF * 32;
  constexpr int SLOT4 = G::SLOT4;
  constexpr int SGN = (MODE == NET_BWD) ? -1 : 1;
  static_assert(KIN % 2 == 0 && NF % 4 == 0 && G::FITS, "shape");

  __shared__ float4 slot0[SLOT4];
  __shared__ float4 slot1[SLOT4];
  __shared__ float epl[6 * F];
  __shared__ float4 k1buf[G::K1BUF4];

  const int tid = threadIdx.x;
  const int lane = tid & 63;
  const int wave = __builtin_amdgcn_readfirstlane(tid >> 6);
  const unsigned voff = (unsigned)lane * 16u;
  const int pix = lane & 31;
  const int hh = lane >> 5;
  const size_t wblk = (size_t)blockIdx.x * 4 + (tid >> 6);
  const int q = (int)wblk * 32 + pix;
  const bool qok = q < a.Q;
  const bool wok = (long)(blockIdx.x * 4 + wave) * 32 < a.Q;
  const float4* ring = a.R0p;

  float xcol[KS1];
  {
    const int hw = a.h * a.w;
    const int qq = qok ? q : 0;
    const int rem = qq % hw;
    const int i = rem / a.w, j = rem % a.w;
    const float* base = a.vin + (long)qq * a.in_stride + a.in_off;
#pragma unroll
    for (int ks = 0; ks < KS1; ++ks) {
      const int k = 2 * ks + hh;
      const int tap = k / KIN, cin = k % KIN;
      const int dy = SGN * (tap / 3 - 1), dx = SGN * (tap % 3 - 1);
      const int ii = i + dy, jj = j + dx;
      const bool ok = qok && ii >= 0 && ii < a.h && jj >= 0 && jj < a.w;
      const int off = ok ? ((dy * a.w + dx) * a.in_stride + cin) : 0;
      const float v = base[off];
      xcol[ks] = ok ? v : 0.0f;
    }
  }
  unsigned mk1[NF / 2], mk2[NF / 2];
#pragma unroll
  for (int j = 0; j < NF / 2; ++j) { mk1[j] = 0; mk2[j] = 0; }
  if (MODE == NET_BWD) {
#pragma unroll
    for (int j = 0; j < NF / 2; ++j) {
      mk1[j] = (unsigned)a.mask1[(wblk * NF + 2 * j) * 64 + lane] | ((unsigned)a.mask1[(wblk * NF + 2 * j + 1) * 64 + lane] << 16);
      mk2[j] = (unsigned)a.mask2[(wblk * NF + 2 * j) * 64 + lane] | ((unsigned)a.mask2[(wblk * NF + 2 * j + 1) * 64 + lane] << 16);
    }
  }
  for (int i = tid; i < 6 * F; i += 256) epl[i] = a.ep[i];
  asm volatile("s_waitcnt vmcnt(0)" ::: "memory");
  stage_range<0, G::PIECES>(ring, slot0, wave, voff);
  if (G::K1_IN_RING) stage_range<NF * 4, (G::K1PIECES > 0 ? G::K1PIECES : 1)>(ring + (size_t)(NF - 1) * SLOT4, slot1, wave, voff);
  else if (G::K1_IN_BUF) stage_range<0, G::K1PIECES_FULL>(reinterpret_cast<const float4*>(a.K1p), k1buf, wave, voff);
  else if (G::K1_IN_HALF) stage_range<0, G::K1HALF_PIECES>(reinterpret_cast<const float4*>(a.K1p), k1buf, wave, voff);

  f32x16 acc2[NF];
#pragma unroll
  for (int fo = 0; fo < NF; ++fo)
#pragma unroll
    for (int r = 0; r < 16; ++r) acc2[fo][r] = 0.0f;

  asm volatile("s_waitcnt vmcnt(0)" ::: "memory");
  __syncthreads();

#pragma nounroll
  for (int fi = 0; fi < NF; fi += 2) {
    net_step<KIN, NF, 0, MODE, STORE>(a, fi, fi == 0, ring + (size_t)(fi + 1) * SLOT4, slot0, slot1, k1buf, epl, xcol, acc2, mk2, wblk, wave, voff, lane, hh, q, qok, wok);
    net_step<KIN, NF, 1, MODE, STORE>(a, fi + 1, false, ring + (size_t)(fi + 2) * SLOT4, slot0, slot1, k1buf, epl, xcol, acc2, mk2, wblk, wave, voff, lane, hh, q, qok, wok);
  }

#pragma unroll
  for (int fo = 0; fo < NF; ++fo) {
    if (MODE == NET_BWD) {
      const unsigned w = mk1[fo >> 1] >> ((fo & 1) * 16);
#pragma unroll
      for (int r = 0; r < 16; ++r) acc2[fo][r] = ((w >> r) & 1u) ? acc2[fo][r] : 0.0f;
      if (STORE && qok) st_tile_planar(uniform_fptr(a.st2 + (size_t)fo * 32 * a.Q), ((unsigned)(4 * hh) * (unsigned)a.Q + (unsigned)q) * 4u, (unsigned)a.Q * 4u, acc2[fo]);
#pragma unroll
      for (int r = 0; r < 16; ++r) acc2[fo][r] *= epl[F + fo * 32 + mfma_row(r, hh)];
    } else {
      unsigned bits = 0;
#pragma unroll
      for (int r = 0; r < 16; ++r) {
        const int f = fo * 32 + mfma_row(r, hh);
        const float pre = acc2[fo][r] + epl[3 * F + f];
        if (MODE == NET_FWD_SAVE) bits |= (pre > 0.0f ? 1u : 0u) << r;
        acc2[fo][r] = fmaxf(pre, 0.0f);
      }
      if (STORE && qok) st_tile_planar(uniform_fptr(a.st2 + (size_t)fo * 32 * a.Q), ((unsigned)(4 * hh) * (unsigned)a.Q + (unsigned)q) * 4u, (unsigned)a.Q * 4u, acc2[fo]);
#pragma unroll
      for (int r = 0; r < 16; ++r) {
        const int f = fo * 32 + mfma_row(r, hh);
        acc2[fo][r] = fmaf(epl[4 * F + f], acc2[fo][r], epl[5 * F + f]);
      }
      if (MODE == NET_FWD_SAVE) a.mask2[(wblk * NF + fo) * 64 + lane] = (unsigned short)bits;
    }
  }

#pragma unroll
  for (int mt = 0; mt < NMT; ++mt) {
    asm volatile("s_waitcnt vmcnt(0)" ::: "memory");
    __syncthreads();
    float4* cur = (mt & 1) ? slot1 : slot0;
    float4* nxt = (mt & 1) ? slot0 : slot1;
    if (mt + 1 < NMT) stage_range<0, NF * 4>(ring + (size_t)(NF + mt + 1) * SLOT4, nxt, wave, voff);
    const float4* buf = cur;
    f32x16 acc3;
#pragma unroll
    for (int r = 0; r < 16; ++r) acc3[r] = 0.0f;
#pragma unroll
    for (int fo = 0; fo < NF; ++fo) {
#pragma unroll
      for (int r4 = 0; r4 < 4; ++r4) {
        const float4 wv = buf[(fo * 4 + r4) * 64 + lane];
// ... 1203 lines not shown
```

### audiosourcesep_amd/csrc/glowk_launch.h

```cpp
#pragma once
#include "glowk_kernels.h"
#include "glowk_co.h"
#include "glowk_q.h"

#include <cstdlib>
#include <string>

#define GLOWK_NET_SHAPES(X) X(2, 16) X(4, 16) X(8, 16) X(16, 16) X(2, 12) X(4, 12) X(8, 12) X(16, 12) \
                            X(2, 8) X(4, 8) X(8, 8) X(16, 8) X(2, 4) X(4, 4) X(8, 4) X(16, 4)

enum NetArith { NET_EXACT, NET_SPLIT3, NET_SPLIT2 };
struct NetCall { int dir; NetArith arith; bool store = false; };

enum NetFamily { FAM_F32, FAM_H3, FAM_H3S, FAM_H3S_HALF, FAM_FUSED, FAM_CO, FAM_Q, FAM_COUNT };

struct NetLaunch {
  int np = 0;
  int family = FAM_F32;
  bool co = false;
  bool q = false;
  int fused_px = 0;
  bool failed = false;
  bool presum = false;
  explicit operator bool() const { return np > 0 || fused_px > 0; }
};

namespace glowk_detail {

int num_cus();
void launch_fail(const std::string&);

struct EnvSwitches {
  bool bwd_light_4;
  bool no_fuse;
  bool wgrad_plain;
  bool co_off;
  bool co_ring3;
  bool q_off;
  bool co_train_off;
  bool train_recompute;
  bool train_perstep;
  bool no_presum;
  bool pg_join;
};
const EnvSwitches& env();

template <int CI, int DIR>
struct NetShape {
  static constexpr int KIN = DIR == NET_BWD ? 2 * CI : CI;
  static constexpr int MOUT = DIR == NET_BWD ? 9 * CI : 18 * CI;
};

template <int CI, int NF, int DIR, bool STORE>
NetLaunch launch_f32(const NetArgs& a, hipStream_t s, bool dry) {
  using Sh = NetShape<CI, DIR>;
  if (!dry) hipLaunchKernelGGL((k_net_f32<Sh::KIN, Sh::MOUT, NF, DIR, STORE>), dim3((a.Q + 127) / 128), dim3(256), 0, s, a);
  return {1, FAM_F32};
}

template <int KIN, int MOUT, int NF, int MODE>
NetLaunch launch_h3(const NetArgs& a, hipStream_t s, bool dry) {
  constexpr bool F2 = RingH<KIN, MOUT, NF, MODE, 2>::FITS, F4 = RingH<KIN, MOUT, NF, MODE, 4>::FITS;
  const int wgs = (a.Q + 255) / 256, cus = num_cus();
  if constexpr (F4) {
    if (a.max_np >= 4 && (4 * wgs <= cus || !F2)) {
      const bool split = 4 * wgs <= cus;
      if (!dry) {
        if (split) hipLaunchKernelGGL((k_net_h3<KIN, MOUT, NF, MODE, 4, true>), dim3(wgs, 4), dim3(512), 0, s, a);
        else hipLaunchKernelGGL((k_net_h3<KIN, MOUT, NF, MODE, 4, false>), dim3(wgs), dim3(512), 0, s, a);
      }
      return {4, FAM_H3};
    }
  }
  if constexpr (F2) {
    if (!dry) {
      if (2 * wgs <= cus) hipLaunchKernelGGL((k_net_h3<KIN, MOUT, NF, MODE, 2, true>), dim3(wgs, 2), dim3(512), 0, s, a);
      else hipLaunchKernelGGL((k_net_h3<KIN, MOUT, NF, MODE, 2, false>), dim3(wgs), dim3(512), 0, s, a);
    }
    return {2, FAM_H3};
  }
  return {};
}

template <class Kernel>
inline bool co_two_per_cu(Kernel kernel) {
  static int blocks = -1;
  if (blocks < 0) {
    int n = 0;
    if (hipOccupancyMaxActiveBlocksPerMultiprocessor(&n, kernel, 256, 0) != hipSuccess) { (void)hipGetLastError(); n = 0; }
    blocks = n;
  }
  return blocks >= 2;
}

template <int KIN, int MOUT, int NF, int MODE>
NetLaunch launch_h3s(const NetArgs& a, hipStream_t s, bool dry) {
  static_assert(!(MODE & NET_STORE), "no storing launches here: the co-resident branch does not check Q % 128 (launch_co_train does)");
  constexpr bool F2 = RingS<KIN, MOUT, NF, MODE, 2>::FITS, F4 = RingS<KIN, MOUT, NF, MODE, 4>::FITS;
  const int wgs = (a.Q + 255) / 256, cus = num_cus();
  if constexpr (F4) {
    if (a.max_np >= 4 && (4 * wgs <= cus || !F2)) {
      const bool split = 4 * wgs <= cus;
      if (!dry) {
        if (split) hipLaunchKernelGGL((k_net_h3s<KIN, MOUT, NF, MODE, 4, true>), dim3(wgs, 4), dim3(512), 0, s, a);
        else hipLaunchKernelGGL((k_net_h3s<KIN, MOUT, NF, MODE, 4, false>), dim3(wgs), dim3(512), 0, s, a);
      }
      return {4, FAM_H3S};
    }
  }
  if constexpr (F2) {
    const bool split = 2 * wgs <= cus;
    if constexpr (RingC<KIN, MOUT, NF, MODE>::FITS) {
      const int wgc = (a.Q + CO_PX - 1) / CO_PX;
      const bool co_ok = a.co && !env().co_off;
      if (co_ok && wgc > cus) {
        if constexpr (RingC<KIN, MOUT, NF, MODE | NET_FUSE>::FITS) {
          if constexpr (RingC<KIN, MOUT, NF, MODE | NET_FUSE>::DB) {
            if (a.fuse && env().co_ring3 && co_two_per_cu(k_net_h3c<KIN, MOUT, NF, MODE | NET_FUSE, false, true>)) {
              if (!dry) hipLaunchKernelGGL((k_net_h3c<KIN, MOUT, NF, MODE | NET_FUSE, false, true>), dim3(wgc), dim3(256), 0, s, a);
              return {0, FAM_FUSED, true, false, CO_PX};
            }
          }
          if (a.fuse && co_two_per_cu(k_net_h3c<KIN, MOUT, NF, MODE | NET_FUSE, false>)) {
            if (!dry) hipLaunchKernelGGL((k_net_h3c<KIN, MOUT, NF, MODE | NET_FUSE, false>), dim3(wgc), dim3(256), 0, s, a);
            return {0, FAM_FUSED, true, false, CO_PX};
          }
        }
        if (!a.fuse && co_two_per_cu(k_net_h3c<KIN, MOUT, NF, MODE, false>)) {
          if (!dry) hipLaunchKernelGGL((k_net_h3c<KIN, MOUT, NF, MODE, false>), dim3(wgc), dim3(256), 0, s, a);
          return {RingC<KIN, MOUT, NF, MODE>::MERGE ? 1 : 2, FAM_H3S, true};
        }
      }
      if (co_ok && split && wgc <= cus && a.max_np >= 2 && co_two_per_cu(k_net_h3c<KIN, MOUT, NF, MODE, true>)) {
        if (!dry) hipLaunchKernelGGL((k_net_h3c<KIN, MOUT, NF, MODE, true>), dim3(wgc, 2), dim3(256), 0, s, a);
        return {2, FAM_H3S, true};
      }
    }
    if constexpr ((MODE == NET_FWD || MODE == NET_FWD2 || MODE == NET_FWD_SAVE) && MOUT == 36) {
      if constexpr (RingS<KIN, MOUT, NF, MODE | NET_FUSE, 2>::FITS && RingS<KIN, MOUT, NF, MODE | NET_FUSE, 2>::MERGE) {
        if (a.fuse && !split) {
          if (!dry) hipLaunchKernelGGL((k_net_h3s<KIN, MOUT, NF, MODE | NET_FUSE, 2, false>), dim3(wgs), dim3(512), 0, s, a);
          return {0, FAM_FUSED, false, false, 256};
        }
      }
    }
    if (!dry) {
      if (split) hipLaunchKernelGGL((k_net_h3s<KIN, MOUT, NF, MODE, 2, true>), dim3(wgs, 2), dim3(512), 0, s, a);
      else hipLaunchKernelGGL((k_net_h3s<KIN, MOUT, NF, MODE, 2, false>), dim3(wgs), dim3(512), 0, s, a);
    }
    return {(!split && RingS<KIN, MOUT, NF, MODE, 2>::MERGE) ? 1 : 2, FAM_H3S};
  }
  return {};
}

inline bool half_wave_grid(const NetArgs& a) { return 8 * ((a.Q + 255) / 256) <= num_cus(); }

template <int KIN, int MOUT, int NF, int MODE>
NetLaunch launch_h3s_half(const NetArgs& a, hipStream_t s, bool dry) {
  if constexpr (RingS<KIN, MOUT, NF, MODE | NET_HALF, 4>::FITS) {
    if (a.max_np < 4) return {};
    const int wgs = (a.Q + 127) / 128;
    if constexpr (RingQ<KIN, MOUT, NF, MODE>::FITS) {
      if (4 * wgs <= num_cus() && !env().q_off) {
        if (!dry) hipLaunchKernelGGL((k_net_h3q<KIN, MOUT, NF, MODE>), dim3(wgs, 4), dim3(512), 0, s, a);
        return {4, FAM_H3S_HALF, false, true};
      }
    }
    if (!dry) {
      if (4 * wgs <= num_cus()) hipLaunchKernelGGL((k_net_h3s<KIN, MOUT, NF, MODE | NET_HALF, 4, true>), dim3(wgs, 4), dim3(512), 0, s, a);
      else hipLaunchKernelGGL((k_net_h3s<KIN, MOUT, NF, MODE | NET_HALF, 4, false>), dim3(wgs), dim3(512), 0, s, a);
    }
    return {4, FAM_H3S_HALF};
  }
  return {};
}

template <int CI, int NF, int STORE = 0>
constexpr bool half_ok() {
  return RingS<CI, 18 * CI, NF, NET_FWD_SAVE | STORE | NET_HALF, 4>::FITS && RingS<2 * CI, 9 * CI, NF, NET_BWD | STORE | NET_HALF, 4>::FITS;
}
template <int CI, int NF>
constexpr bool half_only() {
  return half_ok<CI, NF>() && !(RingS<2 * CI, 9 * CI, NF, NET_BWD, 2>::FITS || RingS<2 * CI, 9 * CI, NF, NET_BWD, 4>::FITS) &&
         !(RingH<2 * CI, 9 * CI, NF, NET_BWD, 2>::FITS || RingH<2 * CI, 9 * CI, NF, NET_BWD, 4>::FITS);
}
template <int CI, int NF>
constexpr bool half_train_only() {
  constexpr int FS = NET_FWD_SAVE | NET_STORE, BS = NET_BWD | NET_STORE;
  return half_ok<CI, NF, NET_STORE>() && !((RingH<CI, 18 * CI, NF, FS, 2>::FITS || RingH<CI, 18 * CI, NF, FS, 4>::FITS) &&
                                           (RingH<2 * CI, 9 * CI, NF, BS, 2>::FITS || RingH<2 * CI, 9 * CI, NF, BS, 4>::FITS));
}
template <int CI, int NF>
inline bool use_half_train(const NetArgs& a) {
  if constexpr (!half_ok<CI, NF, NET_STORE>()) return false;
  return a.fam16 && a.max_np >= 4 && (half_train_only<CI, NF>() || half_wave_grid(a));
}

template <int CI, int NF>
inline bool use_half(const NetArgs& a) {
  if constexpr (!half_ok<CI, NF>()) return false;
  return a.fam16 && a.max_np >= 4 && (half_only<CI, NF>() || half_wave_grid(a));
}

inline bool big_grid(const NetArgs& a) { return 2 * ((a.Q + 255) / 256) > num_cus(); }

template <int CI, int NF>
inline bool co_split_grad(const NetArgs& a) {
  if constexpr (RingC<CI, 18 * CI, NF, NET_FWD_SAVE>::FITS && RingC<2 * CI, 9 * CI, NF, NET_BWD>::FITS) {
    const int wgc = (a.Q + CO_PX - 1) / CO_PX, cus = num_cus();
    return a.co && !env().co_off && a.fam16 && a.max_np >= 2 && 2 * ((a.Q + 255) / 256) <= cus && wgc <= cus &&
           co_two_per_cu(k_net_h3c<CI, 18 * CI, NF, NET_FWD_SAVE, true>) && co_two_per_cu(k_net_h3c<2 * CI, 9 * CI, NF, NET_BWD, true>);
  }
  return false;
}

template <int CI, int NF>
constexpr bool fam16_ok() {
  return RingS<CI, 18 * CI, NF, NET_FWD_SAVE, 2>::FITS && (RingS<2 * CI, 9 * CI, NF, NET_BWD, 2>::FITS || RingS<2 * CI, 9 * CI, NF, NET_BWD, 4>::FITS);
}

template <int CI, int NF, int DIR>
NetLaunch launch_co_train(const NetArgs& a, hipStream_t s, bool dry) {
  constexpr int FS = NET_FWD_SAVE | NET_STORE, BS = NET_BWD | NET_STORE;
  if constexpr (RingC<CI, 18 * CI, NF, FS>::FITS && RingC<2 * CI, 9 * CI, NF, BS>::FITS) {
    const int wgc = (a.Q + CO_PX - 1) / CO_PX, cus = num_cus();
    if (!(a.co && !env().co_off && !env().co_train_off && a.fam16 && a.Q % CO_PX == 0 && a.max_np >= 2)) return {};
    using Sh = NetShape<CI, DIR>;
    if (wgc > cus) {
      if (!(co_two_per_cu(k_net_h3c<CI, 18 * CI, NF, FS, false>) && co_two_per_cu(k_net_h3c<2 * CI, 9 * CI, NF, BS, false>))) return {};
      if (!dry) hipLaunchKernelGGL((k_net_h3c<Sh::KIN, Sh::MOUT, NF, DIR | NET_STORE, false>), dim3(wgc), dim3(256), 0, s, a);
      return {1, FAM_H3S, true};
    }
    if (!(co_two_per_cu(k_net_h3c<CI, 18 * CI, NF, FS, true>) && co_two_per_cu(k_net_h3c<2 * CI, 9 * CI, NF, BS, true>))) return {};
    if (!dry) hipLaunchKernelGGL((k_net_h3c<Sh::KIN, Sh::MOUT, NF, DIR | NET_STORE, true>), dim3(wgc, 2), dim3(256), 0, s, a);
    return {2, FAM_H3S, true};
  }
  return {};
}

template <int CI, int NF>
NetLaunch launch_split3_fwd(const NetArgs& a, bool half, hipStream_t s, bool dry) {
  NetLaunch r;
  if (half && a.RSp && half_wave_grid(a) && !a.fuse) r = launch_h3s_half<CI, 18 * CI, NF, NET_FWD>(a, s, dry);
  if (!r && a.RSp) r = launch_h3s<CI, 18 * CI, NF, NET_FWD>(a, s, dry);
  if (!r && a.RHp) r = launch_h3<CI, 18 * CI, NF, NET_FWD>(a, s, dry);
  if (!r) r = launch_f32<CI, NF, NET_FWD, false>(a, s, dry);
  return r;
}
template <int CI, int NF>
NetLaunch launch_split2_fwd(const NetArgs& a, hipStream_t s, bool dry) {
  NetLaunch r;
  if (a.RSp) r = launch_h3s<CI, 18 * CI, NF, NET_FWD2>(a, s, dry);
  return r ? r : launch_split3_fwd<CI, NF>(a, false, s, dry);
}

template <int CI, int NF, int DIR>
NetLaunch launch_split_grad(const NetArgs& a, hipStream_t s, bool dry) {
  using Sh = NetShape<CI, DIR>;
  NetLaunch r;
  if (use_half<CI, NF>(a)) r = launch_h3s_half<Sh::KIN, Sh::MOUT, NF, DIR>(a, s, dry);
  if constexpr (fam16_ok<CI, NF>()) {
    if (!r && a.fam16 && (big_grid(a) || co_split_grad<CI, NF>(a))) r = launch_h3s<Sh::KIN, Sh::MOUT, NF, DIR>(a, s, dry);
  }
  if (!r && a.RHp) r = launch_h3<Sh::KIN, Sh::MOUT, NF, DIR>(a, s, dry);
  if (!r) r = launch_f32<CI, NF, DIR, false>(a, s, dry);
  return r;
}

inline NetLaunch net_failed(const std::string& m) { launch_fail(m); NetLaunch r; r.failed = true; return r; }

template <int CI, int NF, int DIR>
NetLaunch launch_split_train(const NetArgs& a, hipStream_t s, bool dry) {
  using Sh = NetShape<CI, DIR>;
  constexpr int MODE = DIR | NET_STORE;
  NetLaunch r;
  if (use_half_train<CI, NF>(a)) r = launch_h3s_half<Sh::KIN, Sh::MOUT, NF, MODE>(a, s, dry);
  if (!r) r = launch_co_train<CI, NF, DIR>(a, s, dry);
  if (!r && a.RHp) r = launch_h3<Sh::KIN, Sh::MOUT, NF, MODE>(a, s, dry);
  if (!r && !dry) return net_failed("no split-arithmetic training instance for this shape");
  return r;
}

template <int CI, int NF, bool STORE>
NetLaunch launch_exact(const NetArgs& a, int dir, hipStream_t s, bool dry) {
  if (dir == NET_FWD) return launch_f32<CI, NF, NET_FWD, STORE>(a, s, dry);
  if (dir == NET_FWD_SAVE) return launch_f32<CI, NF, NET_FWD_SAVE, STORE>(a, s, dry);
  return launch_f32<CI, NF, NET_BWD, STORE>(a, s, dry);
}

template <int CI, int NF>
NetLaunch launch_net_t(const NetArgs& a, NetCall call, hipStream_t s, bool dry) {
  const bool save = call.dir == NET_FWD_SAVE;
  if (call.dir != NET_FWD && !save && call.dir != NET_BWD) return net_failed("bad k_net mode");
  NetLaunch r;
  if (call.arith == NET_EXACT) {
    r = !call.store ? launch_exact<CI, NF, false>(a, call.dir, s, dry) : launch_exact<CI, NF, true>(a, call.dir, s, dry);
  } else if (call.store) {
    if (call.dir == NET_FWD || call.arith != NET_SPLIT3) return net_failed("bad k_net mode");
    r = save ? launch_split_train<CI, NF, NET_FWD_SAVE>(a, s, dry) : launch_split_train<CI, NF, NET_BWD>(a, s, dry);
  } else if (call.dir == NET_FWD) {
    r = call.arith == NET_SPLIT3 ? launch_split3_fwd<CI, NF>(a, true, s, dry) : launch_split2_fwd<CI, NF>(a, s, dry);
  } else {
    if (call.arith != NET_SPLIT3) return net_failed("bad k_net mode");
    r = save ? launch_split_grad<CI, NF, NET_FWD_SAVE>(a, s, dry) : launch_split_grad<CI, NF, NET_BWD>(a, s, dry);
  }
  if (!dry && !r.failed) {
    hipError_t e = hipGetLastError();
    if (e != hipSuccess) return net_failed(std::string("k_net: ") + hipGetErrorString(e));
  }
  r.presum = a.pw != 0 && call.dir != NET_BWD && (r.family == FAM_H3S || r.family == FAM_H3S_HALF) && RingS<CI, 18 * CI, NF, NET_FWD, 2>::C3P;
  return r;
}

}
```

### audiosourcesep_amd/engine.py

```python
import ctypes
import os
import warnings

import numpy as np
import torch

from . import _lib
from .config import GlowConfig


def _stream_ptr(device):
    return ctypes.c_void_p(torch.cuda.current_stream(device).cuda_stream)


def _ptr(t):
    return ctypes.c_void_p(t.data_ptr()) if t is not None else ctypes.c_void_p(0)


class GlowEngine:
    _reserved_grad = 0
    _grad_cap = None
    _ran_grad = 0
    _grad_chunk = (None, 0)

    def __init__(self, cfg: GlowConfig, device=None):
        self.lib = _lib.load()
        if not torch.cuda.is_available():
            raise RuntimeError("glowk needs a ROCm GPU (torch.cuda.is_available() is False); there is no CPU path")
        self.cfg = cfg
        self.device = torch.device("cuda", torch.cuda.current_device() if device is None else device)
        c = _lib.GlowkConfigStruct(cfg.H, cfg.W, cfg.C, cfg.L, cfg.K, cfg.F, int(cfg.learntop), int(cfg.use_logit),
                                   cfg.minval, cfg.maxval, cfg.alpha, cfg.bn_eps)
        h = ctypes.c_void_p()
        _lib.check(self.lib.glowk_create(ctypes.byref(c), self.device.index, ctypes.byref(h)))
        self.h = h
        self._finalized = False
        self._max_tiles_cap = None
        self._fallbacks_seen = 0
        self.set_range_policy("fallback")

    def _stream(self):
        return _stream_ptr(self.device)

    def close(self):
        if getattr(self, "h", None):
            self.lib.glowk_destroy(self.h)
            self.h = None

    def __del__(self):
        try:
            self.close()
        except Exception:
            pass

    @staticmethod
    def _split_name(name):
        if name in _lib.PRIOR_TENSOR_IDS:
            return -1, 0, _lib.PRIOR_TENSOR_IDS[name]
        lvl, stp, rest = name.split("/", 2)
        return int(lvl[1:]), int(stp[1:]), _lib.STEP_TENSOR_IDS[rest]

    def set_tensor(self, name, value):
        level, step, tid = self._split_name(name)
        a = np.ascontiguousarray(np.asarray(value, dtype=np.float32)).ravel()
        _lib.check(self.lib.glowk_set_tensor(self.h, level, step, tid, a.ctypes.data_as(_lib._fp), a.size))
        self._finalized = False

    def get_tensor(self, name):
        level, step, tid = self._split_name(name)
        n = self.lib.glowk_tensor_size(self.h, level, tid)
        a = np.empty(n, dtype=np.float32)
        _lib.check(self.lib.glowk_get_tensor(self.h, level, step, tid, a.ctypes.data_as(_lib._fp), a.size))
        return a

    def load_params(self, params):
        for name, value in params.items():
            self.set_tensor(name, value)
        self.finalize()

    def finalize(self):
        _lib.check(self.lib.glowk_finalize_weights(self.h))
        self._finalized = True

    def actnorm_data_init(self, minibatch, runtime_order=False, raw_minibatch_quirk=True):
        x = self._in(minibatch, self.data_shape)
        _lib.check(self.lib.glowk_actnorm_data_init(self.h, _ptr(x), x.shape[0], int(runtime_order), int(raw_minibatch_quirk),
                                                    self._stream()))

    def actnorm_params(self):
        out = {}
        for lvl in range(self.cfg.L):
            for k in range(self.cfg.K):
                for t in ("actnorm/log_scale", "actnorm/shift"):
                    name = "b%d/s%d/%s" % (lvl, k, t)
                    out[name] = self.get_tensor(name)
        return out

    def set_precision(self, mode):
        _lib.check(self.lib.glowk_set_precision(self.h, int(mode)))

    def get_precision(self):
        return int(self.lib.glowk_get_precision(self.h))

    def set_range_policy(self, policy):
        modes = {"ignore": _lib.RANGE_IGNORE, "error": _lib.RANGE_ERROR, "fallback": _lib.RANGE_FALLBACK}
        _lib.check(self.lib.glowk_set_range_policy(self.h, modes[policy] if isinstance(policy, str) else int(policy)))

    def range_status(self, sync=True):
        tripped, n = ctypes.c_int(0), ctypes.c_int64(0)
        _lib.check(self.lib.glowk_range_status(self.h, ctypes.byref(tripped) if sync else None, ctypes.byref(n), self._stream()))
        return bool(tripped.value), int(n.value)

    def range_probe_begin(self):
        _lib.check(self.lib.glowk_range_probe_begin(self.h))

    def range_probe_end(self):
        f, b = ctypes.c_float(0), ctypes.c_float(0)
        _lib.check(self.lib.glowk_range_probe_end(self.h, ctypes.byref(f), ctypes.byref(b), self._stream()))
        return float(f.value), float(b.value)

    def _after_call(self):
        if self.get_precision() == _lib.PREC_F32:
            return
        n = self.range_status(sync=False)[1]
        if n > self._fallbacks_seen:
            if self._fallbacks_seen == 0:
                warnings.warn("glowk: a hidden activation left the fp16 range of the split arithmetic; the call was re-run on the "
                              "exact fp32 kernels (slower). Consider set_precision(PREC_F32) for this checkpoint.", RuntimeWarning,
                              stacklevel=3)
            self._fallbacks_seen = n

    def reserve(self, n, with_grad=False):
        m = min(int(n), self.grad_max_tiles if with_grad else self.max_tiles)
        self._reserve_or_shrink(m, with_grad)

    def _reserve_or_shrink(self, m, with_grad):
        while True:
            try:
                _lib.check(self.lib.glowk_reserve(self.h, int(m), int(with_grad)))
                break
            except _lib.GlowkError as e:
                if not with_grad or m <= 1 or "out of memory" not in str(e).lower():
                    raise
                torch.cuda.empty_cache()
                m = max(1, m // 2)
                self._reserved_grad = 0
                self._ran_grad = 0
                self._grad_cap = m
        if with_grad:
            self._reserved_grad = max(self._reserved_grad, int(m))

    @property
    def max_tiles(self):
        m = int(self.lib.glowk_max_tiles(self.h))
        return min(m, self._max_tiles_cap) if self._max_tiles_cap else m

    def _chunks(self, n, m=None):
        m = m or self.max_tiles
        return [(i, min(i + m, n)) for i in range(0, n, m)]

    @property
    def grad_max_tiles(self):
        if not self._finalized:
            self.finalize()
        free = self._free_bytes()
        own = self.workspace_bytes(self._reserved_grad, True) if self._reserved_grad else 0
        key = (self.get_precision(), self._max_tiles_cap, (free + own) >> 30)
        key = key + (self._grad_cap,)
        if self._grad_chunk[0] == key:
            return self._grad_chunk[1]
        budget = min(0.6 * (free + own), float(os.environ.get("GLOWK_GRAD_BUDGET_GB", "64")) * 2 ** 30)
        top = min(self.max_tiles, self._grad_cap or self.max_tiles)
        lo, hi = 1, top
        if self.workspace_bytes(hi, True) > budget:
            while lo < hi:
                mid = (lo + hi + 1) // 2
                if self.workspace_bytes(mid, True) <= budget:
                    lo = mid
                else:
                    hi = mid - 1
        else:
            lo = hi
        lo = max(lo, min(self._ran_grad, top))
        self._grad_chunk = (key, lo)
        return lo

    def _free_bytes(self):
        return torch.cuda.mem_get_info(self.device)[0]

    def workspace_bytes(self, n, with_grad=False):
        return int(self.lib.glowk_workspace_bytes(self.h, int(n), int(with_grad)))

    @property
    def fused_steps(self):
        return int(self.lib.glowk_fused_steps(self.h))

    def kernel_families(self):
        out = (ctypes.c_int64 * 7)()
        _lib.check(self.lib.glowk_kernel_families(self.h, out))
        return dict(zip(("f32", "h3_32x32x16", "h3s_16x16x32", "h3s_half", "fused", "co_resident", "small_grid_q"), [int(v) for v in out]))

    def profile_begin(self):
        _lib.check(self.lib.glowk_profile_begin(self.h))

    def profile_end(self):
        p = _lib.GlowkProfile()
        _lib.check(self.lib.glowk_profile_end(self.h, ctypes.byref(p)))
        return [(p.net_ms[i], int(p.net_launches[i])) for i in range(self.cfg.L)]

    def _in(self, x, shape_tail):
        if not torch.is_tensor(x):
            x = torch.as_tensor(np.asarray(x, dtype=np.float32))
        x = x.to(device=self.device, dtype=torch.float32).contiguous()
        if tuple(x.shape[1:]) != tuple(shape_tail):
            raise ValueError("expected a [N, %s] tensor, got %s" % (", ".join(map(str, shape_tail)), tuple(x.shape)))
        if not self._finalized:
            self.finalize()
        return x

    def _new(self, *shape):
        return torch.empty(shape, device=self.device, dtype=torch.float32)

    @property
    def data_shape(self):
        return (self.cfg.H, self.cfg.W, self.cfg.C)

    def _compute(self, rc):
        _lib.check(rc)
        self._after_call()

    def forward(self, x, with_logdet=True):
        x = self._in(x, self.data_shape)
        n = x.shape[0]
        z = self._new(n, *self.cfg.latent_shape())
        ld = self._new(n) if with_logdet else None
        if n == 0:
            return (z, ld) if with_logdet else z
        for a, b in self._chunks(n):
            self._compute(self.lib.glowk_forward(self.h, _ptr(x[a:b]), b - a, _ptr(z[a:b]), _ptr(ld[a:b] if with_logdet else None),
                                              self._stream()))
        return (z, ld) if with_logdet else z

    def inverse(self, z):
        z = self._in(z, self.cfg.latent_shape())
        n = z.shape[0]
        x = self._new(n, *self.data_shape)
        if n == 0:
            return x
        for a, b in self._chunks(n):
            self._compute(self.lib.glowk_inverse(self.h, _ptr(z[a:b]), b - a, _ptr(x[a:b]), self._stream()))
        return x

    def log_prob(self, x, return_latent=False, out=None):
        x = self._in(x, self.data_shape)
        n = x.shape[0]
        lp = out if out is not None else self._new(n)
        z = self._new(n, *self.cfg.latent_shape()) if return_latent else None
        if n == 0:
            return (lp, z) if return_latent else lp
        for a, b in self._chunks(n):
            self._compute(self.lib.glowk_log_prob(self.h, _ptr(x[a:b]), b - a, _ptr(lp[a:b]), _ptr(z[a:b] if return_latent else None),
                                               self._stream()))
        return (lp, z) if return_latent else lp

    def log_prob_sum(self, x, out=None, total=None):
        x = self._in(x, self.data_shape)
        n = x.shape[0]
        lp = out if out is not None else self._new(n)
        if total is None:
            total = torch.empty(1, device=self.device, dtype=torch.float64)
        if n == 0:
            _lib.check(self.lib.glowk_sum_f64(_ptr(None), 0, _ptr(total), 0, 1.0, self._stream()))
            return lp, total
        for i, (a, b) in enumerate(self._chunks(n)):
            self._compute(self.lib.glowk_log_prob_sum(self.h, _ptr(x[a:b]), b - a, _ptr(lp[a:b]), _ptr(None), _ptr(total), int(i > 0),
                                                   self._stream()))
        return lp, total

    def sum_f64(self, v, scale=1.0, out=None):
        v = v.contiguous()
        if out is None:
            out = torch.empty(1, device=v.device, dtype=torch.float64)
        _lib.check(self.lib.glowk_sum_f64(_ptr(v), v.numel(), _ptr(out), 0, float(scale), _stream_ptr(v.device)))
        return out

    def log_prob_grad(self, x):
        x = self._in(x, self.data_shape)
        n = x.shape[0]
        lp, dx = self._new(n), torch.empty_like(x)
        if n == 0:
            return lp, dx
        chunk = self.grad_max_tiles
        if min(n, chunk) > self._reserved_grad:
            self._reserve_or_shrink(min(n, chunk), True)
            chunk = min(chunk, self.grad_max_tiles)
        for a, b in self._chunks(n, chunk):
            self._compute(self.lib.glowk_log_prob_grad(self.h, _ptr(x[a:b]), b - a, _ptr(lp[a:b]), _ptr(dx[a:b]), self._stream()))
        self._ran_grad = max(self._ran_grad, min(n, chunk))
        return lp, dx

    @property
    def param_vector_size(self):
        return int(self.lib.glowk_param_vector_size(self.h))

    def param_slice(self, name):
        level, step, tid = self._split_name(name)
        off, cnt = ctypes.c_size_t(0), ctypes.c_size_t(0)
        _lib.check(self.lib.glowk_param_offset(self.h, level, step, tid, ctypes.byref(off), ctypes.byref(cnt)))
        return int(off.value), int(cnt.value)

    def param_grad(self, x, scale, grad=None):
        x = self._in(x, self.data_shape)
        n = x.shape[0]
        if n > self.grad_max_tiles:
            raise ValueError("param_grad takes at most %d tiles per call (split the batch and add the gradients)" % self.grad_max_tiles)
        lp = self._new(n)
        if grad is None:
            grad = self._new(self.param_vector_size)
        self._compute(self.lib.glowk_param_grad(self.h, _ptr(x), n, float(scale), _ptr(lp), _ptr(grad), self._stream()))
        if n > self._ran_grad:
            self._ran_grad = n
            self._grad_chunk = (None, 0)
        return lp, grad

    def apply_gradients(self, grad, optimizer="adamax", lr=1e-3):
        opt = {"adam": 0, "adamax": 1}
        if optimizer not in opt:
            raise ValueError("optimizer argument should be adam or adamax")
        _lib.check(self.lib.glowk_apply_gradients(self.h, _ptr(grad), opt[optimizer], float(lr), self._stream()))
        self._finalized = True

    def sample_from_eps(self, eps):
        eps = self._in(eps, self.cfg.latent_shape())
        n = eps.shape[0]
        x = self._new(n, *self.data_shape)
        if n == 0:
            return x
        for a, b in self._chunks(n):
            self._compute(self.lib.glowk_sample(self.h, _ptr(eps[a:b]), b - a, _ptr(x[a:b]), self._stream()))
        return x

    def prior_log_prob(self, z):
        z = self._in(z, self.cfg.latent_shape())
        lp = self._new(z.shape[0])
        for a, b in self._chunks(z.shape[0]):
            _lib.check(self.lib.glowk_prior_log_prob(self.h, _ptr(z[a:b]), b - a, _ptr(lp[a:b]), self._stream()))
        return lp

    def preprocess_forward(self, x):
        x = self._in(x, self.data_shape)
        y, ld = torch.empty_like(x), self._new(x.shape[0])
        _lib.check(self.lib.glowk_preprocess_forward(self.h, _ptr(x), x.shape[0], _ptr(y), _ptr(ld), self._stream()))
        return y, ld

    def preprocess_inverse(self, y):
        y = self._in(y, self.data_shape)
        x = torch.empty_like(y)
        _lib.check(self.lib.glowk_preprocess_inverse(self.h, _ptr(y), y.shape[0], _ptr(x), self._stream()))
        return x

    def step_forward(self, level, step, u):
        u = self._in(u, self.cfg.level_shapes()[level])
        y, ld = torch.empty_like(u), self._new(u.shape[0])
        self._compute(self.lib.glowk_step_forward(self.h, level, step, _ptr(u), u.shape[0], _ptr(y), _ptr(ld), self._stream()))
        return y, ld

    def step_inverse(self, level, step, y):
        y = self._in(y, self.cfg.level_shapes()[level])
        u = torch.empty_like(y)
        self._compute(self.lib.glowk_step_inverse(self.h, level, step, _ptr(y), y.shape[0], _ptr(u), self._stream()))
        return u

    def coupling_net(self, level, step, xb):
        h, w, c = self.cfg.level_shapes()[level]
        xb = self._in(xb, (h, w, c // 2))
        log_s, t = torch.empty_like(xb), torch.empty_like(xb)
        self._compute(self.lib.glowk_coupling_net(self.h, level, step, _ptr(xb), xb.shape[0], _ptr(log_s), _ptr(t), self._stream()))
        return log_s, t


def squeeze(x):
    lib = _lib.load()
    x = x.contiguous()
    n, H, W, C = x.shape
    y = torch.empty((n, H // 2, W // 2, 4 * C), device=x.device, dtype=torch.float32)
    _lib.check(lib.glowk_squeeze(_ptr(x), n, H, W, C, _ptr(y), _stream_ptr(x.device)))
    return y


def unsqueeze(y):
    lib = _lib.load()
    y = y.contiguous()
    n, h, w, c4 = y.shape
    x = torch.empty((n, 2 * h, 2 * w, c4 // 4), device=y.device, dtype=torch.float32)
    _lib.check(lib.glowk_unsqueeze(_ptr(y), n, h, w, c4, _ptr(x), _stream_ptr(y.device)))
    return x
```

### include/glowk.h

```cpp
#ifndef GLOWK_H
#define GLOWK_H

#include <stddef.h>
#include <stdint.h>

#ifdef __cplusplus
extern "C" {
#endif

#define GLOWK_VERSION 480

typedef struct glowk_config {
  int32_t H, W, C;
  int32_t L, K, F;
  int32_t learntop;
  int32_t use_logit;
  float minval, maxval, alpha;
  float bn_eps;
} glowk_config;

typedef struct glowk_handle glowk_handle;

enum glowk_tensor_id {
  GLOWK_ACTNORM_LOG_SCALE = 0,
  GLOWK_ACTNORM_SHIFT = 1,
  GLOWK_INV1X1_P = 2,
  GLOWK_INV1X1_SIGN_S = 3,
  GLOWK_INV1X1_L = 4,
  GLOWK_INV1X1_LOG_S = 5,
  GLOWK_INV1X1_U = 6,
  GLOWK_CONV1_KERNEL = 7,
  GLOWK_CONV1_BIAS = 8,
  GLOWK_BN1_GAMMA = 9,
  GLOWK_BN1_BETA = 10,
  GLOWK_BN1_MEAN = 11,
  GLOWK_BN1_VAR = 12,
  GLOWK_CONV2_KERNEL = 13,
  GLOWK_CONV2_BIAS = 14,
  GLOWK_BN2_GAMMA = 15,
  GLOWK_BN2_BETA = 16,
  GLOWK_BN2_MEAN = 17,
  GLOWK_BN2_VAR = 18,
  GLOWK_CONV3_KERNEL = 19,
  GLOWK_CONV3_BIAS = 20,
  GLOWK_INV1X1_P_INV = 21,
  GLOWK_NUM_STEP_TENSORS = 22,
  GLOWK_PRIOR_LOC = 100,
  GLOWK_PRIOR_LOG_SCALE = 101
};

enum glowk_precision {
  GLOWK_PREC_F32 = 0,
  GLOWK_PREC_F16X3 = 1,
  GLOWK_PREC_F16X2 = 2
};

enum glowk_status {
  GLOWK_OK = 0,
  GLOWK_ERR = 1,
  GLOWK_ERR_RANGE = 2
};

enum glowk_range_policy { GLOWK_RANGE_IGNORE = 0, GLOWK_RANGE_ERROR = 1, GLOWK_RANGE_FALLBACK = 2 };

int glowk_version(void);
const char* glowk_last_error(void);
void glowk_reload_env(void);

int glowk_create(const glowk_config* cfg, int device, glowk_handle** out);
int glowk_destroy(glowk_handle* h);
size_t glowk_tensor_size(const glowk_handle* h, int level, int tensor_id);
int glowk_set_tensor(glowk_handle* h, int level, int step, int tensor_id, const float* host, size_t n);
int glowk_get_tensor(const glowk_handle* h, int level, int step, int tensor_id, float* host, size_t n);
int glowk_finalize_weights(glowk_handle* h);
int glowk_actnorm_data_init(glowk_handle* h, const float* x_dev, int N, int runtime_order, int raw_minibatch_quirk, void* stream);
int glowk_set_precision(glowk_handle* h, int precision);
int glowk_get_precision(const glowk_handle* h);
int glowk_set_range_policy(glowk_handle* h, int policy);
int glowk_get_range_policy(const glowk_handle* h);
int glowk_range_status(glowk_handle* h, int* tripped, int64_t* fallbacks, void* stream);
int glowk_range_probe_begin(glowk_handle* h);
int glowk_range_probe_end(glowk_handle* h, float* fwd_ratio, float* bwd_ratio, void* stream);
size_t glowk_workspace_bytes(const glowk_handle* h, int N, int with_grad);
int glowk_reserve(glowk_handle* h, int N, int with_grad);
int glowk_max_tiles(const glowk_handle* h);

int glowk_forward(glowk_handle* h, const float* x_dev, int N, float* z_dev, float* logdet_dev, void* stream);
int glowk_inverse(glowk_handle* h, const float* z_dev, int N, float* x_dev, void* stream);
int glowk_log_prob(glowk_handle* h, const float* x_dev, int N, float* logp_dev, float* z_dev, void* stream);
int glowk_log_prob_sum(glowk_handle* h, const float* x_dev, int N, float* logp_dev, float* z_dev, double* sum_dev, int accumulate,
                       void* stream);
int glowk_sum_f64(const float* v_dev, size_t n, double* out_dev, int accumulate, double scale, void* stream);
int glowk_log_prob_grad(glowk_handle* h, const float* x_dev, int N, float* logp_dev, float* dx_dev, void* stream);
int glowk_sample(glowk_handle* h, const float* eps_dev, int N, float* x_dev, void* stream);
int glowk_prior_log_prob(glowk_handle* h, const float* z_dev, int N, float* logp_dev, void* stream);

typedef struct glowk_profile {
  double net_ms[4];
  int64_t net_launches[4];
} glowk_profile;
int glowk_profile_begin(glowk_handle* h);
int64_t glowk_fused_steps(const glowk_handle* h);
int glowk_kernel_families(const glowk_handle* h, int64_t* out7);
int glowk_profile_end(glowk_handle* h, glowk_profile* out);

int glowk_squeeze(const float* x_dev, int N, int H, int W, int C, float* y_dev, void* stream);
int glowk_unsqueeze(const float* y_dev, int N, int h, int w, int c4, float* x_dev, void* stream);
int glowk_preprocess_forward(glowk_handle* h, const float* x_dev, int N, float* y_dev, float* logdet_dev, void* stream);
int glowk_preprocess_inverse(glowk_handle* h, const float* y_dev, int N, float* x_dev, void* stream);
int glowk_step_forward(glowk_handle* h, int level, int step, const float* u_dev, int N, float* y_dev, float* logdet_dev, void* stream);
int glowk_step_inverse(glowk_handle* h, int level, int step, const float* y_dev, int N, float* u_dev, void* stream);
int glowk_coupling_net(glowk_handle* h, int level, int step, const float* xb_dev, int N, float* log_s_dev, float* t_dev, void* stream);

size_t glowk_param_vector_size(glowk_handle* h);
int glowk_param_offset(glowk_handle* h, int level, int step, int tensor_id, size_t* offset, size_t* count);
int glowk_param_grad(glowk_handle* h, const float* x_dev, int N, float scale, float* logp_dev, float* grad_dev, void* stream);
int glowk_apply_gradients(glowk_handle* h, const float* grad_dev, int optimizer, float lr, void* stream);

int glowk_basis_update(float* x1_dev, float* x2_dev, const float* g1_dev, const float* g2_dev, const float* mixed_dev, size_t n,
                       float eta, float lambda_recon, const float* eps1_dev, const float* eps2_dev, uint64_t seed, uint64_t step,
                       uint64_t offset, int* nonfinite_dev, void* stream);
int glowk_basis_mix(const float* x1_dev, const float* x2_dev, float* out_dev, size_t n, void* stream);
enum glowk_mixing {
  GLOWK_MIX_DB = 0,
  GLOWK_MIX_MEAN = 1
};
int glowk_basis_update_n(float* const* x, const float* const* g, const float* const* eps, int nsrc, const float* mixed_dev, size_t n,
                         int mixing, float eta, float lambda_recon, uint64_t seed, uint64_t step, uint64_t offset,
                         int* nonfinite_dev, void* stream);
int glowk_basis_mix_n(const float* const* x, int nsrc, float* out_dev, size_t n, int mixing, void* stream);
int glowk_random(float* out_dev, size_t n, uint64_t seed, uint64_t step, int which, int uniform, uint64_t offset, void* stream);
int glowk_random_source(float* out_dev, size_t n, uint64_t seed, uint64_t step, int which, int pair, int uniform, uint64_t offset,
                        void* stream);
int glowk_add_noise(const float* x_dev, float* out_dev, size_t n, float sigma, uint64_t seed, uint64_t step, int which, uint64_t offset,
                    void* stream);

int glowk_mel_filterbank(float* host_out);
int glowk_mel_frontend(const float* audio_dev, int N, int n_samples, float top_db, float* mel_db_dev, float* stft_dev, void* stream);
int glowk_mel_to_power(const float* mel_db_dev, int N, int frames, int iters, float* power_dev, void* stream);
int glowk_masked_istft(const float* power_dev, int S, const float* stft_mix_dev, int N, int frames, int wiener, float* audio_dev,
                       void* stream);
int glowk_griffinlim(const float* mag_dev, const float* angles0_dev, int N, int frames, int n_iter, float momentum, float* audio_dev,
                     void* stream);

int64_t glowk_resample_length(int64_t n_in, int sr_in, int sr_out);
int glowk_resample_filter(double* host_out);
int glowk_resample(const float* x_dev, int nsig, int64_t n_in, int sr_in, int sr_out, float* y_dev, void* stream);

int glowk_bss_xcorr(const double* sig_dev, int nsig, int64_t nsampl, const int64_t* win_dev, int nwin, int64_t max_len, const int* pairs_dev,
                    int npairs, int filters_len, double* corr_dev, void* stream);
int glowk_bss_solve(const double* corr_dev, int nwin, int npairs, int nref, int filters_len, int nchan_sys, const int* sys_dev, int nsys,
                    double* coef_dev, int* status_dev, void* stream);
int glowk_bss_project(const double* sig_dev, int64_t nsampl, int nsrc, int nchan, int filters_len, const int64_t* items_dev, int nitems,
                      int64_t max_len, const double* coef_c_dev, int nsys_c, const double* coef_j_dev, int nsys_j, double* energy_dev,
                      void* stream);

int glowk_sp_stft(const float* x_dev, int nsig, int64_t n, float* spec_dev, void* stream);
int glowk_sp_istft(const float* spec_dev, int nsig, int frames, int64_t length, float* out_dev, void* stream);
int glowk_oracle_mask(float* spec_dev, int nsrc, int nchan, int frames, int irm, double alpha, double theta, uint8_t* mask_dev,
                      void* stream);
int glowk_mwf(float* spec_dev, int nsrc, int frames, void* stream);
int glowk_oracle_mel(const double* mix_dev, const void* src_dev, int nsrc, int64_t n, int src_f64, int irm, double theta, void* out_dev,
                     void* stream);

int glowk_mwf_em(const float* x_dev, float* v_dev, int nsrc, int nprob, int frames, int n_iter, float* y_dev, double* r_dev,
                 void* stream);

int glowk_mel_frames(const float* audio_dev, int nsig, int64_t n_samples, float* mel_db_dev, float* stft_dev, void* stream);
int glowk_tile_cut(const float* frames_dev, int nsig, int frames, int width, int hop, float top_db, float* tiles_dev, void* stream);
int glowk_tile_stitch(const float* tiles_dev, int nsig, int N, int width, int hop, int frames, float* frames_dev, void* stream);

uint32_t glowk_crc32c(const void* host_data, size_t n);

#ifdef __cplusplus
}
#endif
#endif
```

Before: 16950.

## Split forward pass into sub-batches run concurrently on forked streams

For large batches, the forward pass is partitioned into up to four sub-batches (default two). Each sub-batch runs the level and step chain on its own stream, with a fork event and join events, so kernels from different chunks can overlap and fill gaps between dependent launches. Each sub-batch gets its own scratch region in bufP, and kernel-selection heuristics use the whole-call Q so every chunk picks the same variant. The cost is extra stream and event overhead and smaller per-launch grids, which could lower per-kernel efficiency.

```diff
diff --git a/audiosourcesep_amd/_lib.py b/audiosourcesep_amd/_lib.py
--- a/audiosourcesep_amd/_lib.py
+++ b/audiosourcesep_amd/_lib.py
@@ -79,6 +79,7 @@
     "glowk_sample": (_i, [_vp, _vp, _i, _vp, _vp]),
     "glowk_prior_log_prob": (_i, [_vp, _vp, _i, _vp, _vp]),
     "glowk_fused_steps": (ctypes.c_int64, [_vp]),
+    "glowk_subbatch_calls": (ctypes.c_int64, [_vp]),
     "glowk_kernel_families": (_i, [_vp, ctypes.POINTER(ctypes.c_int64)]),
     "glowk_profile_begin": (_i, [_vp]),
     "glowk_profile_end": (_i, [_vp, ctypes.POINTER(GlowkProfile)]),
diff --git a/audiosourcesep_amd/csrc/glowk.hip b/audiosourcesep_amd/csrc/glowk.hip
--- a/audiosourcesep_amd/csrc/glowk.hip
+++ b/audiosourcesep_amd/csrc/glowk.hip
@@ -1,5 +1,6 @@
 #include "glowk_engine.h"
 #include "glowk_light.h"
+#include "glowk_subbatch.h"
 
 namespace glowk_eng {
 thread_local std::string g_err;
@@ -21,10 +22,19 @@
   return n;
 }
 void launch_fail(const std::string& m) { fail(m); }
+constexpr int SUBBATCH_DEFAULT = 2, SUBBATCH_FROM_DEFAULT = 0;
 static EnvSwitches read_env() {
   auto on = [](const char* n) { return getenv(n) != nullptr; };
+  auto num = [](const char* n, int lo, int hi, int dflt) {
+    const char* v = getenv(n);
+    if (!v || !*v) return dflt;
+    char* end = nullptr;
+    const long x = strtol(v, &end, 10);
+    return (*end || x < lo || x > hi) ? dflt : (int)x;
+  };
   return EnvSwitches{on("GLOWK_BWD_LIGHT_4"), on("GLOWK_NO_FUSE"), on("GLOWK_WGRAD_PLAIN"), on("GLOWK_CO_OFF"), on("GLOWK_CO_RING3"), on("GLOWK_Q_OFF"), on("GLOWK_CO_TRAIN_OFF"),
-                     on("GLOWK_TRAIN_RECOMPUTE"), on("GLOWK_TRAIN_PERSTEP"), on("GLOWK_NO_PRESUM"), on("GLOWK_PG_JOIN")};
+                     on("GLOWK_TRAIN_RECOMPUTE"), on("GLOWK_TRAIN_PERSTEP"), on("GLOWK_NO_PRESUM"), on("GLOWK_PG_JOIN"),
+                     num("GLOWK_SUBBATCH", 1, glowk_sub::MAX_PARTS, SUBBATCH_DEFAULT), num("GLOWK_SUBBATCH_FROM", 0, 1, SUBBATCH_FROM_DEFAULT)};
 }
 static EnvSwitches g_env = read_env();
 const EnvSwitches& env() { return g_env; }
@@ -59,7 +69,7 @@
   return glowk_detail::net_failed("unsupported (channels, n_filters) combination: c=" + std::to_string(c) + " F=" + std::to_string(F));
 }
 
-int launch_net(glowk_handle* h, int level, int c, int F, const NetArgs& a, hipStream_t s, NetCall call, NetLaunch* out = nullptr) {
+int launch_net(glowk_handle* h, int level, int c, int F, const NetArgs& a, hipStream_t s, NetCall call, NetLaunch* out = nullptr, int sub = 0) {
   if (h->profiling) {
     while (h->ev_pool.size() < h->ev_used + 2) {
       OwnedEvent e;
@@ -69,7 +79,7 @@
     HIPCHK(hipEventRecord(h->ev_pool[h->ev_used], s));
   }
   const NetLaunch r = launch_net_raw(c, F, a, call, s);
-  if (!r.failed) {
+  if (!r.failed && sub <= 1) {
     ++h->family_launches[r.family];
     if (r.co) ++h->family_launches[FAM_CO];
     if (r.q) ++h->family_launches[FAM_Q];
@@ -78,6 +88,7 @@
     HIPCHK(hipEventRecord(h->ev_pool[h->ev_used + 1], s));
     h->ev_used += 2;
     h->ev_level.push_back(level);
+    h->ev_sub.push_back((unsigned char)sub);
   }
   if (out) *out = r;
   return r.failed ? 1 : 0;
@@ -105,8 +116,10 @@
     default: return fail("pre-summed P at channel count " + std::to_string(c));                \
   }
 
-int launch_couple(int c, const CoupleArgs& a, int N, hipStream_t s, const FlatLd* fl = nullptr, bool* flat_used = nullptr) {
+int launch_couple(int c, const CoupleArgs& a, int N, hipStream_t s, const FlatLd* fl = nullptr, bool* flat_used = nullptr, int n_sub = 0) {
   const int hw = a.h * a.w;
+  if (n_sub > 0 && N < 2 * num_cus()) return fail("sub-batched coupling launch below 2 x CUs tiles");
+  const int ng = n_sub > 0 ? n_sub : N;
   if (N < 2 * num_cus() && hw % 64 == 0 && (!a.logdet || (fl && fl->slot))) {
     CoupleArgs b = a;
     b.logdet = nullptr;
@@ -123,8 +136,8 @@
     return 0;
   }
   if (N >= 2 * num_cus()) {
-    if (a.presum) { PDISPATCH(c, hipLaunchKernelGGL((k_couple<CC, false, true>), dim3(N), dim3(256), 0, s, a)); }
-    else { CDISPATCH(c, hipLaunchKernelGGL((k_couple<CC, false>), dim3(N), dim3(256), 0, s, a)); }
+    if (a.presum) { PDISPATCH(c, hipLaunchKernelGGL((k_couple<CC, false, true>), dim3(ng), dim3(256), 0, s, a)); }
+    else { CDISPATCH(c, hipLaunchKernelGGL((k_couple<CC, false>), dim3(ng), dim3(256), 0, s, a)); }
   } else {
     const int threads = hw >= 256 ? 1024 : hw > 64 ? 512 : 256;
     if (a.presum) { PDISPATCH(c, hipLaunchKernelGGL((k_couple<CC, true, true>), dim3(N), dim3(threads), 0, s, a)); }
@@ -141,40 +154,48 @@
   return hw >= 32 && hw < pxw && (hw & (hw - 1)) == 0;
 }
 
+struct SubLaunch {
+  int sub = 0;
+  int n = 0;
+  size_t p_off = 0;
+  size_t region_floats = 0;
+};
 int net_and_couple(glowk_handle* h, int lvl, int c, int F, NetArgs na, CoupleArgs ca, int N, hipStream_t s, NetCall call, const FlatLd* fl = nullptr,
-                   bool* flat_used = nullptr) {
+                   bool* flat_used = nullptr, const SubLaunch* sb = nullptr) {
+  float* const pbase = h->bufP + (sb ? sb->p_off : 0);
   const bool no_fuse = glowk_detail::env().no_fuse;
   const bool fusable = call.arith != NET_EXACT && call.dir != NET_BWD && !call.store;
   const int hw = ca.h * ca.w;
   if (!no_fuse && c == 4 && fusable && na.RSp && ca.vin && !ca.log_s_out && ca.out && na.in_stride == 4 &&
-      ca.out_stride % 4 == 0 && ca.out_off % 4 == 0 && fuse_geometry_ok(ca.h, ca.w) && na.P == h->bufP) {
+      ca.out_stride % 4 == 0 && ca.out_off % 4 == 0 && fuse_geometry_ok(ca.h, ca.w) && na.P == pbase) {
     const size_t pxw = (na.co && fuse_geometry_ok(ca.h, ca.w, CO_PX)) ? CO_PX : 256;
     if (pxw == 256) na.co = 0;
-    const size_t wgs = ((size_t)ca.Q + pxw - 1) / pxw;
-    const size_t edge_floats = (wgs * 4 * FUSE_EW * 4 + 3) & ~(size_t)3;
-    const size_t nld = wgs * (pxw / 32);
-    if ((edge_floats + 2 * nld + 4) <= 4 * h->pstride) {
+    static_assert(glowk_sub::FUSE_EDGE_W == FUSE_EW, "glowk_subbatch.h sizes the edge slots");
+    const glowk_sub::FuseScratch fs = glowk_sub::fuse_scratch((size_t)ca.Q, pxw);
+    const size_t edge_floats = fs.edge_floats;
+    if (glowk_sub::fuse_scratch_fits(fs, !sb, sb ? sb->region_floats : 0, h->pstride)) {
       na.fuse = 1;
       na.fz_b3 = ca.b3; na.fz_A = ca.A; na.fz_b = ca.b; na.fz_out = ca.out; na.fz_out_stride = ca.out_stride; na.fz_out_off = ca.out_off;
       na.fz_inverse = ca.inverse;
       na.fz_osave = ca.o_save;
-      na.fz_edge = h->bufP;
-      na.fz_ldpart = ca.logdet ? reinterpret_cast<double*>(h->bufP + edge_floats) : nullptr;
+      na.fz_edge = pbase;
+      na.fz_ldpart = ca.logdet ? reinterpret_cast<double*>(pbase + edge_floats) : nullptr;
     }
   }
   NetLaunch r;
-  if (int rc = launch_net(h, lvl, c, F, na, s, call, &r)) return rc;
+  const int ng = sb ? sb->n : N;
+  if (int rc = launch_net(h, lvl, c, F, na, s, call, &r, sb ? sb->sub : 0)) return rc;
   if (!r.fused_px) {
     ca.P = na.P; ca.np = r.np; ca.pstride = na.pstride; ca.presum = r.presum ? 1 : 0;
-    return launch_couple(c, ca, N, s, fl, flat_used);
-  }
-  ++h->fused_steps;
+    return launch_couple(c, ca, N, s, fl, flat_used, sb ? sb->n : 0);
+  }
+  if (!sb || sb->sub <= 1) ++h->fused_steps;
   const int pxw = r.fused_px;
   if (hw > pxw || ca.logdet) {
     EdgeArgs ea;
     ea.vin = ca.vin; ea.edge = na.fz_edge; ea.ldpart = na.fz_ldpart; ea.A = ca.A; ea.b = ca.b; ea.out = ca.out; ea.out_stride = ca.out_stride;
     ea.out_off = ca.out_off; ea.inverse = ca.inverse; ea.logdet = ca.logdet; ea.osave = ca.o_save; ea.h = ca.h; ea.w = ca.w; ea.flag = ca.flag; ea.pxw = pxw;
-    hipLaunchKernelGGL(k_couple_edge, dim3(N), dim3(256), 0, s, ea);
+    hipLaunchKernelGGL(k_couple_edge, dim3(ng), dim3(256), 0, s, ea);
     LAUNCHCHK("k_couple_edge");
   }
   return 0;
@@ -309,7 +330,7 @@
   a.fuse = 0; a.co = glowk_detail::env().co_off ? 0 : 1; a.fz_osave = nullptr; a.fz_b3 = nullptr; a.fz_A = nullptr; a.fz_b = nullptr; a.fz_out = nullptr; a.fz_out_stride = 0; a.fz_out_off = 0; a.fz_inverse = 0;
   a.fz_edge = nullptr; a.fz_ldpart = nullptr;
   a.pw = (!glowk_detail::env().no_presum && (lv.c == 8 || lv.c == 16) && lv.w >= 4 && lv.w <= 16 && (lv.w & (lv.w - 1)) == 0) ? lv.w : 0;
-  a.pad = 0;
+  a.Qcall = 0;
   a.xmax_out = h->d_probe ? h->d_probe + ((&lv - h->levels.data()) * h->cfg.K + (&sd - lv.dev.data())) : nullptr;
   return a;
 }
@@ -329,69 +350,142 @@
   return 0;
 }
 
+int ensure_subbatch(glowk_handle* h, int S) {
+  if ((int)h->sb_streams.size() >= S - 1) return 0;
+  std::vector<OwnedStream> streams(glowk_sub::MAX_PARTS - 1);
+  std::vector<OwnedEvent> joins(glowk_sub::MAX_PARTS - 1);
+  OwnedEvent fork;
+  for (OwnedStream& t : streams) HIPCHK(stream_create(t));
+  for (OwnedEvent& e : joins) HIPCHK(event_create(e, hipEventDisableTiming));
+  HIPCHK(event_create(fork, hipEventDisableTiming));
+  h->sb_streams = std::move(streams);
+  h->sb_joins = std::move(joins);
+  h->sb_fork = std::move(fork);
+  return 0;
+}
+
 int run_forward(glowk_handle* h, const float* x, int N, float* z_dst, hipStream_t s, bool save, bool keep_hidden) {
   const glowk_config& cfg = h->cfg;
   const int K = cfg.K, L = cfg.L, NF = cfg.F / 32;
-  float* cur = save ? h->saveV + h->offV[0] : h->bufA;
-  float* oth = h->bufB;
   const int nslots = ld_slots_per_sample(h);
   const NetCall call = net_call(h, save ? NET_FWD_SAVE : NET_FWD, keep_hidden);
   const bool flat_ok = N < 2 * num_cus() && h->bufLdSlot;
   bool flat_used = false;
   int slot_base = 0;
   if (flat_ok) HIPCHK(hipMemsetAsync(h->bufLdSlot, 0, (size_t)N * nslots * 8, s));
-  {
-    const Level& lv = h->levels[0];
-    const StepDev& first = lv.dev[K - 1];
-    CDISPATCH(lv.c, hipLaunchKernelGGL((k_in<CC>), dim3(N), dim3(256), 0, s, x, cfg.H, cfg.W, pre_args(cfg), 1,
-                                       first.Afwd, first.bfwd, cur, h->bufLd, h->ld_const + h->ld_pre_const));
-    LAUNCHCHK("k_in");
-  }
-  for (int lvl = 0; lvl < L; ++lvl) {
-    const Level& lv = h->levels[lvl];
-    const size_t Q = (size_t)N * lv.h * lv.w;
-    const size_t blocks = mask_blocks(lv, Q);
-    for (int k = K - 1; k >= 0; --k) {
-      const StepDev& sd = lv.dev[k];
-      const size_t sidx = (size_t)lvl * K + (K - 1 - k);
-      NetArgs na = net_args(h, lv, sd, cur, lv.c, lv.c / 2, N);
-      if (save) {
-        na.mask1 = h->saveM + h->offM[sidx];
-        na.mask2 = na.mask1 + blocks * NF * 64;
+
+  const size_t E = (size_t)cfg.H * cfg.W * cfg.C;
+  const glowk_detail::EnvSwitches& ev = glowk_detail::env();
+  glowk_sub::Partition parts = glowk_sub::partition(N, num_cus(), (save || keep_hidden) ? 1 : ev.subbatch);
+  const int from = ev.subbatch_from;
+  if (parts.S > 1 && from >= L) parts = glowk_sub::partition(N, num_cus(), 1);
+  if (parts.S > 1 && (size_t)N * glowk_sub::tile_floats(E) > h->pstride) parts = glowk_sub::partition(N, num_cus(), 1);
+  for (int i = 0; i < parts.S && parts.S > 1; ++i) {
+    const Level& l0 = h->levels[0];
+    const glowk_sub::FuseScratch fs = glowk_sub::fuse_scratch((size_t)parts.part[i].n * l0.h * l0.w, CO_PX);
+    if (!glowk_sub::fuse_scratch_fits(fs, false, glowk_sub::p_region_floats(parts.part[i], E), h->pstride)) parts = glowk_sub::partition(N, num_cus(), 1);
+  }
+  const int S = parts.S;
+  if (S > 1) {
+    if (int rc = ensure_subbatch(h, S)) return rc;
+    ++h->subbatch_calls;
+  }
+
+  struct Chain { float* cur; float* oth; int slot_base; };
+  auto run_levels = [&](Chain& ch, int l0, int l1, bool with_in, const glowk_sub::Part& pt, int sub, hipStream_t st) -> int {
+    const int n0 = pt.n0, n = pt.n;
+    double* const ld = h->bufLd + n0;
+    float* const zd = z_dst + (size_t)n0 * h->Hl * h->Wl * h->Cl;
+    SubLaunch sl;
+    sl.sub = sub; sl.n = n; sl.p_off = glowk_sub::p_region_off(pt, E); sl.region_floats = glowk_sub::p_region_floats(pt, E);
+    const SubLaunch* sb = sub ? &sl : nullptr;
+    if (with_in) {
+      const Level& lv = h->levels[0];
+      const StepDev& first = lv.dev[K - 1];
+      CDISPATCH(lv.c, hipLaunchKernelGGL((k_in<CC>), dim3(n), dim3(256), 0, st, x + (size_t)n0 * E, cfg.H, cfg.W, pre_args(cfg), 1,
+                                         first.Afwd, first.bfwd, ch.cur + (size_t)n0 * lv.h * lv.w * lv.c, ld, h->ld_const + h->ld_pre_const));
+      LAUNCHCHK("k_in");
+    }
+    for (int lvl = l0; lvl < l1; ++lvl) {
+      const Level& lv = h->levels[lvl];
+      const size_t Q = (size_t)n * lv.h * lv.w;
+      const size_t toff = (size_t)n0 * lv.h * lv.w * lv.c;
+      const size_t blocks = mask_blocks(lv, Q);
+      for (int k = K - 1; k >= 0; --k) {
+        const StepDev& sd = lv.dev[k];
+        const size_t sidx = (size_t)lvl * K + (K - 1 - k);
+        float* const cur = ch.cur + toff;
+        float* const oth = ch.oth + toff;
+        NetArgs na = net_args(h, lv, sd, cur, lv.c, lv.c / 2, n);
+        if (sb) { na.Qcall = N * lv.h * lv.w; na.P = h->bufP + sl.p_off; }
+        if (save) {
+          na.mask1 = h->saveM + h->offM[sidx];
+          na.mask2 = na.mask1 + blocks * NF * 64;
+        }
+        if (keep_hidden) {
+          na.st1 = h->trKeep + h->trKeepOff[sidx] * (size_t)N;
+          na.st2 = na.st1 + (size_t)cfg.F * Q;
+        }
+        CoupleArgs ca;
+        ca.presum = 0;
+        ca.vin = cur; ca.b3 = sd.b3; ca.logdet = ld; ca.log_s_out = nullptr; ca.t_out = nullptr;
+        ca.o_save = save ? h->saveP + h->offP[sidx] : nullptr;
+        ca.Q = (int)Q; ca.h = lv.h; ca.w = lv.w; ca.inverse = 0; ca.flag = flagp(h);
+        float* next = save && k > 0 ? h->saveV + h->offV[sidx + 1] : oth;
+        if (k > 0) {
+          ca.A = lv.dev[k - 1].Afwd; ca.b = lv.dev[k - 1].bfwd;
+          ca.out = next; ca.out_stride = lv.c; ca.out_off = 0;
+        } else if (lvl < L - 1) {
+          ca.A = nullptr; ca.b = nullptr; ca.out = oth; ca.out_stride = lv.c; ca.out_off = 0;
+        } else {
+          ca.A = nullptr; ca.b = nullptr; ca.out = zd; ca.out_stride = h->Cl; ca.out_off = lv.z_off;
+        }
+        const FlatLd fl{flat_ok ? h->bufLdSlot : nullptr, nslots, ch.slot_base};
+        ch.slot_base += (lv.h * lv.w + 15) / 16;
+        if (int rc = net_and_couple(h, lvl, lv.c, cfg.F, na, ca, N, st, call, &fl, &flat_used, sb)) return rc;
+        if (k > 0) {
+          if (save) ch.cur = next; else std::swap(ch.cur, ch.oth);
+        } else if (lvl < L - 1) {
+          const Level& nl = h->levels[lvl + 1];
+          float* nvb = save ? h->saveV + h->offV[sidx + 1] : ch.cur;
+          float* nv = nvb + (size_t)n0 * nl.h * nl.w * nl.c;
+          const StepDev& nfirst = nl.dev[K - 1];
+          CDISPATCH(lv.c, hipLaunchKernelGGL((k_split<CC>), dim3(n), dim3(256), 0, st, (const float*)oth, lv.h, lv.w, zd, h->Hl * h->Wl, h->Cl,
+                                             lv.z_off, lv.Cz, nfirst.Afwd, nfirst.bfwd, nv));
+          LAUNCHCHK("k_split");
+          ch.cur = nvb;
+          if (!save) ch.oth = (ch.cur == h->bufA) ? h->bufB : h->bufA;
+        }
       }
-      if (keep_hidden) {
-        na.st1 = h->trKeep + h->trKeepOff[sidx] * (size_t)N;
-        na.st2 = na.st1 + (size_t)cfg.F * Q;
+    }
+    return 0;
+  };
+
+  Chain ch{save ? h->saveV + h->offV[0] : (float*)h->bufA, (float*)h->bufB, slot_base};
+  const glowk_sub::Part whole{0, N};
+  if (S == 1) {
+    if (int rc = run_levels(ch, 0, L, true, whole, 0, s)) return rc;
+  } else {
+    if (from > 0)
+      if (int rc = run_levels(ch, 0, from, true, whole, 0, s)) return rc;
+    HIPCHK(hipEventRecord(h->sb_fork, s));
+    int rc = 0;
+    int forked = 0;
+    for (int i = 0; i < S && !rc; ++i) {
+      hipStream_t st = i == 0 ? s : (hipStream_t)h->sb_streams[i - 1];
+      if (i > 0) {
+        if (hipStreamWaitEvent(st, h->sb_fork, 0) != hipSuccess) { rc = fail("hipStreamWaitEvent(fork) failed"); break; }
+        forked = i;
       }
-      CoupleArgs ca;
-      ca.presum = 0;
-      ca.vin = cur; ca.b3 = sd.b3; ca.logdet = h->bufLd; ca.log_s_out = nullptr; ca.t_out = nullptr;
-      ca.o_save = save ? h->saveP + h->offP[sidx] : nullptr;
-      ca.Q = (int)Q; ca.h = lv.h; ca.w = lv.w; ca.inverse = 0; ca.flag = flagp(h);
-      float* next = save && k > 0 ? h->saveV + h->offV[sidx + 1] : oth;
-      if (k > 0) {
-        ca.A = lv.dev[k - 1].Afwd; ca.b = lv.dev[k - 1].bfwd;
-        ca.out = next; ca.out_stride = lv.c; ca.out_off = 0;
-      } else if (lvl < L - 1) {
-        ca.A = nullptr; ca.b = nullptr; ca.out = oth; ca.out_stride = lv.c; ca.out_off = 0;
-      } else {
-        ca.A = nullptr; ca.b = nullptr; ca.out = z_dst; ca.out_stride = h->Cl; ca.out_off = lv.z_off;
-      }
-      const FlatLd fl{flat_ok ? h->bufLdSlot : nullptr, nslots, slot_base};
-      slot_base += (lv.h * lv.w + 15) / 16;
-      if (int rc = net_and_couple(h, lvl, lv.c, cfg.F, na, ca, N, s, call, &fl, &flat_used)) return rc;
-      if (k > 0) {
-        if (save) cur = next; else std::swap(cur, oth);
-      } else if (lvl < L - 1) {
-        float* nv = save ? h->saveV + h->offV[sidx + 1] : cur;
-        const StepDev& nfirst = h->levels[lvl + 1].dev[K - 1];
-        CDISPATCH(lv.c, hipLaunchKernelGGL((k_split<CC>), dim3(N), dim3(256), 0, s, (const float*)oth, lv.h, lv.w, z_dst, h->Hl * h->Wl, h->Cl,
-                                           lv.z_off, lv.Cz, nfirst.Afwd, nfirst.bfwd, nv));
-        LAUNCHCHK("k_split");
-        cur = nv;
-        if (!save) oth = (cur == h->bufA) ? h->bufB : h->bufA;
-      }
-    }
+      Chain ci = ch;
+      rc = run_levels(ci, from, L, from == 0, parts.part[i], i + 1, st);
+    }
+    for (int i = 1; i <= forked; ++i) {
+      hipError_t e = hipEventRecord(h->sb_joins[i - 1], h->sb_streams[i - 1]);
+      if (e == hipSuccess) e = hipStreamWaitEvent(s, h->sb_joins[i - 1], 0);
+      if (e != hipSuccess && !rc) rc = fail(std::string("joining the sub-batch chains: ") + hipGetErrorString(e));
+    }
+    if (rc) return rc;
   }
   if (flat_used) {
     hipLaunchKernelGGL(k_ld_fold, dim3(N), dim3(64), 0, s, h->bufLd, (const double*)h->bufLdSlot, nslots);
@@ -1074,6 +1168,7 @@
 }
 
 int64_t glowk_fused_steps(const glowk_handle* h) { return h ? h->fused_steps : -1; }
+int64_t glowk_subbatch_calls(const glowk_handle* h) { return h ? h->subbatch_calls : -1; }
 
 int glowk_kernel_families(const glowk_handle* h, int64_t* out7) {
   if (!h || !out7) return fail("null argument");
@@ -1086,6 +1181,7 @@
   h->profiling = true;
   h->ev_used = 0;
   h->ev_level.clear();
+  h->ev_sub.clear();
   return 0;
 }
 
@@ -1095,14 +1191,44 @@
   h->profiling = false;
   DeviceGuard dg(h->device);
   HIPCHK(hipDeviceSynchronize());
+  bool subbed[4] = {false, false, false, false};
+  for (size_t i = 0; i < h->ev_level.size(); ++i)
+    if (h->ev_sub[i] && h->ev_level[i] >= 0 && h->ev_level[i] < 4) subbed[h->ev_level[i]] = true;
+  std::vector<std::pair<float, float>> iv[4];
   for (size_t i = 0; i < h->ev_level.size(); ++i) {
-    float ms = 0.0f;
-    HIPCHK(hipEventElapsedTime(&ms, h->ev_pool[2 * i], h->ev_pool[2 * i + 1]));
     const int l = h->ev_level[i];
-    if (l >= 0 && l < 4) { out->net_ms[l] += ms; out->net_launches[l] += 1; }
-  }
+    if (l < 0 || l >= 4) continue;
+    if (h->ev_sub[i] <= 1) out->net_launches[l] += 1;
+    if (!subbed[l]) {
+      float ms = 0.0f;
+      HIPCHK(hipEventElapsedTime(&ms, h->ev_pool[2 * i], h->ev_pool[2 * i + 1]));
+      out->net_ms[l] += ms;
+    } else {
+      float t0 = 0.0f, t1 = 0.0f;
+      if (i > 0) HIPCHK(hipEventElapsedTime(&t0, h->ev_pool[0], h->ev_pool[2 * i]));
+      HIPCHK(hipEventElapsedTime(&t1, h->ev_pool[0], h->ev_pool[2 * i + 1]));
+      iv[l].emplace_back(t0, std::max(t0, t1));
+    }
+  }
+  std::vector<std::pair<float, int>> edges;
+  for (int l = 0; l < 4; ++l)
+    for (const std::pair<float, float>& v : iv[l]) { edges.emplace_back(v.first, l + 1); edges.emplace_back(v.second, -(l + 1)); }
+  std::sort(edges.begin(), edges.end());
+  int active[4] = {0, 0, 0, 0};
+  double acc[4] = {0.0, 0.0, 0.0, 0.0};
+  for (size_t j = 0; j < edges.size(); ++j) {
+    if (j > 0) {
+      const double dt = (double)edges[j].first - (double)edges[j - 1].first;
+      for (int l = 0; l < 4; ++l)
+        if (active[l] > 0) { acc[l] += dt; break; }
+    }
+    if (edges[j].second > 0) ++active[edges[j].second - 1]; else --active[-edges[j].second - 1];
+  }
+  for (int l = 0; l < 4; ++l)
+    if (!iv[l].empty()) out->net_ms[l] = acc[l];
   h->ev_used = 0;
   h->ev_level.clear();
+  h->ev_sub.clear();
   return 0;
 }
 
diff --git a/audiosourcesep_amd/csrc/glowk_engine.h b/audiosourcesep_amd/csrc/glowk_engine.h
--- a/audiosourcesep_amd/csrc/glowk_engine.h
+++ b/audiosourcesep_amd/csrc/glowk_engine.h
@@ -103,6 +103,7 @@
   int64_t range_fallbacks = 0;
   int64_t family_launches[FAM_COUNT] = {};
   int64_t fused_steps = 0;
+  int64_t subbatch_calls = 0;
   DeviceMem<int> d_flag;
   PinnedMem<int> h_flag;
   DeviceMem<unsigned> d_probe;
@@ -165,6 +166,10 @@
   std::vector<OwnedEvent> ev_pool;
   size_t ev_used = 0;
   std::vector<int> ev_level;
+  std::vector<unsigned char> ev_sub;
+  std::vector<OwnedStream> sb_streams;
+  std::vector<OwnedEvent> sb_joins;
+  OwnedEvent sb_fork;
 };
 
 #define CDISPATCH(c, CALL)                                                                     \
diff --git a/audiosourcesep_amd/csrc/glowk_kernels.h b/audiosourcesep_amd/csrc/glowk_kernels.h
--- a/audiosourcesep_amd/csrc/glowk_kernels.h
+++ b/audiosourcesep_amd/csrc/glowk_kernels.h
@@ -46,7 +46,7 @@
   float* st1;
   float* st2;
   int pw;
-  int pad;
+  int Qcall;
 };
 static_assert(sizeof(NetArgs) == 264, "kernel argument size");
 
diff --git a/audiosourcesep_amd/csrc/glowk_launch.h b/audiosourcesep_amd/csrc/glowk_launch.h
--- a/audiosourcesep_amd/csrc/glowk_launch.h
+++ b/audiosourcesep_amd/csrc/glowk_launch.h
@@ -42,6 +42,8 @@
   bool train_perstep;
   bool no_presum;
   bool pg_join;
+  int subbatch;
+  int subbatch_from;
 };
 const EnvSwitches& env();
 
@@ -51,6 +53,8 @@
   static constexpr int MOUT = DIR == NET_BWD ? 9 * CI : 18 * CI;
 };
 
+inline int policy_q(const NetArgs& a) { return a.Qcall > 0 ? a.Qcall : a.Q; }
+
 template <int CI, int NF, int DIR, bool STORE>
 NetLaunch launch_f32(const NetArgs& a, hipStream_t s, bool dry) {
   using Sh = NetShape<CI, DIR>;
@@ -61,10 +65,10 @@
 template <int KIN, int MOUT, int NF, int MODE>
 NetLaunch launch_h3(const NetArgs& a, hipStream_t s, bool dry) {
   constexpr bool F2 = RingH<KIN, MOUT, NF, MODE, 2>::FITS, F4 = RingH<KIN, MOUT, NF, MODE, 4>::FITS;
-  const int wgs = (a.Q + 255) / 256, cus = num_cus();
+  const int wgs = (a.Q + 255) / 256, wgp = (policy_q(a) + 255) / 256, cus = num_cus();
   if constexpr (F4) {
-    if (a.max_np >= 4 && (4 * wgs <= cus || !F2)) {
-      const bool split = 4 * wgs <= cus;
+    if (a.max_np >= 4 && (4 * wgp <= cus || !F2)) {
+      const bool split = 4 * wgp <= cus;
       if (!dry) {
         if (split) hipLaunchKernelGGL((k_net_h3<KIN, MOUT, NF, MODE, 4, true>), dim3(wgs, 4), dim3(512), 0, s, a);
         else hipLaunchKernelGGL((k_net_h3<KIN, MOUT, NF, MODE, 4, false>), dim3(wgs), dim3(512), 0, s, a);
@@ -74,7 +78,7 @@
   }
   if constexpr (F2) {
     if (!dry) {
-      if (2 * wgs <= cus) hipLaunchKernelGGL((k_net_h3<KIN, MOUT, NF, MODE, 2, true>), dim3(wgs, 2), dim3(512), 0, s, a);
+      if (2 * wgp <= cus) hipLaunchKernelGGL((k_net_h3<KIN, MOUT, NF, MODE, 2, true>), dim3(wgs, 2), dim3(512), 0, s, a);
       else hipLaunchKernelGGL((k_net_h3<KIN, MOUT, NF, MODE, 2, false>), dim3(wgs), dim3(512), 0, s, a);
     }
     return {2, FAM_H3};
@@ -97,10 +101,10 @@
 NetLaunch launch_h3s(const NetArgs& a, hipStream_t s, bool dry) {
   static_assert(!(MODE & NET_STORE), "no storing launches here: the co-resident branch does not check Q % 128 (launch_co_train does)");
   constexpr bool F2 = RingS<KIN, MOUT, NF, MODE, 2>::FITS, F4 = RingS<KIN, MOUT, NF, MODE, 4>::FITS;
-  const int wgs = (a.Q + 255) / 256, cus = num_cus();
+  const int wgs = (a.Q + 255) / 256, wgp = (policy_q(a) + 255) / 256, cus = num_cus();
   if constexpr (F4) {
-    if (a.max_np >= 4 && (4 * wgs <= cus || !F2)) {
-      const bool split = 4 * wgs <= cus;
+    if (a.max_np >= 4 && (4 * wgp <= cus || !F2)) {
+      const bool split = 4 * wgp <= cus;
       if (!dry) {
         if (split) hipLaunchKernelGGL((k_net_h3s<KIN, MOUT, NF, MODE, 4, true>), dim3(wgs, 4), dim3(512), 0, s, a);
         else hipLaunchKernelGGL((k_net_h3s<KIN, MOUT, NF, MODE, 4, false>), dim3(wgs), dim3(512), 0, s, a);
@@ -109,11 +113,11 @@
     }
   }
   if constexpr (F2) {
-    const bool split = 2 * wgs <= cus;
+    const bool split = 2 * wgp <= cus;
     if constexpr (RingC<KIN, MOUT, NF, MODE>::FITS) {
-      const int wgc = (a.Q + CO_PX - 1) / CO_PX;
+      const int wgc = (a.Q + CO_PX - 1) / CO_PX, wgcp = (policy_q(a) + CO_PX - 1) / CO_PX;
       const bool co_ok = a.co && !env().co_off;
-      if (co_ok && wgc > cus) {
+      if (co_ok && wgcp > cus) {
         if constexpr (RingC<KIN, MOUT, NF, MODE | NET_FUSE>::FITS) {
           if constexpr (RingC<KIN, MOUT, NF, MODE | NET_FUSE>::DB) {
             if (a.fuse && env().co_ring3 && co_two_per_cu(k_net_h3c<KIN, MOUT, NF, MODE | NET_FUSE, false, true>)) {
@@ -131,7 +135,7 @@
           return {RingC<KIN, MOUT, NF, MODE>::MERGE ? 1 : 2, FAM_H3S, true};
         }
       }
-      if (co_ok && split && wgc <= cus && a.max_np >= 2 && co_two_per_cu(k_net_h3c<KIN, MOUT, NF, MODE, true>)) {
+      if (co_ok && split && wgcp <= cus && a.max_np >= 2 && co_two_per_cu(k_net_h3c<KIN, MOUT, NF, MODE, true>)) {
         if (!dry) hipLaunchKernelGGL((k_net_h3c<KIN, MOUT, NF, MODE, true>), dim3(wgc, 2), dim3(256), 0, s, a);
         return {2, FAM_H3S, true};
       }
@@ -153,21 +157,21 @@
   return {};
 }
 
-inline bool half_wave_grid(const NetArgs& a) { return 8 * ((a.Q + 255) / 256) <= num_cus(); }
+inline bool half_wave_grid(const NetArgs& a) { return 8 * ((policy_q(a) + 255) / 256) <= num_cus(); }
 
 template <int KIN, int MOUT, int NF, int MODE>
 NetLaunch launch_h3s_half(const NetArgs& a, hipStream_t s, bool dry) {
   if constexpr (RingS<KIN, MOUT, NF, MODE | NET_HALF, 4>::FITS) {
     if (a.max_np < 4) return {};
-    const int wgs = (a.Q + 127) / 128;
+    const int wgs = (a.Q + 127) / 128, wgp = (policy_q(a) + 127) / 128;
     if constexpr (RingQ<KIN, MOUT, NF, MODE>::FITS) {
-      if (4 * wgs <= num_cus() && !env().q_off) {
+      if (4 * wgp <= num_cus() && !env().q_off) {
         if (!dry) hipLaunchKernelGGL((k_net_h3q<KIN, MOUT, NF, MODE>), dim3(wgs, 4), dim3(512), 0, s, a);
         return {4, FAM_H3S_HALF, false, true};
       }
     }
     if (!dry) {
-      if (4 * wgs <= num_cus()) hipLaunchKernelGGL((k_net_h3s<KIN, MOUT, NF, MODE | NET_HALF, 4, true>), dim3(wgs, 4), dim3(512), 0, s, a);
+      if (4 * wgp <= num_cus()) hipLaunchKernelGGL((k_net_h3s<KIN, MOUT, NF, MODE | NET_HALF, 4, true>), dim3(wgs, 4), dim3(512), 0, s, a);
       else hipLaunchKernelGGL((k_net_h3s<KIN, MOUT, NF, MODE | NET_HALF, 4, false>), dim3(wgs), dim3(512), 0, s, a);
     }
     return {4, FAM_H3S_HALF};
@@ -202,13 +206,13 @@
   return a.fam16 && a.max_np >= 4 && (half_only<CI, NF>() || half_wave_grid(a));
 }
 
-inline bool big_grid(const NetArgs& a) { return 2 * ((a.Q + 255) / 256) > num_cus(); }
+inline bool big_grid(const NetArgs& a) { return 2 * ((policy_q(a) + 255) / 256) > num_cus(); }
 
 template <int CI, int NF>
 inline bool co_split_grad(const NetArgs& a) {
   if constexpr (RingC<CI, 18 * CI, NF, NET_FWD_SAVE>::FITS && RingC<2 * CI, 9 * CI, NF, NET_BWD>::FITS) {
-    const int wgc = (a.Q + CO_PX - 1) / CO_PX, cus = num_cus();
-    return a.co && !env().co_off && a.fam16 && a.max_np >= 2 && 2 * ((a.Q + 255) / 256) <= cus && wgc <= cus &&
+    const int wgc = (policy_q(a) + CO_PX - 1) / CO_PX, cus = num_cus();
+    return a.co && !env().co_off && a.fam16 && a.max_np >= 2 && 2 * ((policy_q(a) + 255) / 256) <= cus && wgc <= cus &&
            co_two_per_cu(k_net_h3c<CI, 18 * CI, NF, NET_FWD_SAVE, true>) && co_two_per_cu(k_net_h3c<2 * CI, 9 * CI, NF, NET_BWD, true>);
   }
   return false;
diff --git a/audiosourcesep_amd/csrc/glowk_subbatch.h b/audiosourcesep_amd/csrc/glowk_subbatch.h
--- /dev/null
+++ b/audiosourcesep_amd/csrc/glowk_subbatch.h
@@ -0,0 +1,41 @@
+#pragma once
+#include <cstddef>
+
+namespace glowk_sub {
+
+constexpr int MAX_PARTS = 4;
+constexpr size_t FUSE_EDGE_W = 64;
+
+struct Part { int n0, n; };
+struct Partition { int S; Part part[MAX_PARTS]; };
+
+inline Partition partition(int N, int cus, int want) {
+  Partition p{};
+  int S = want < 1 ? 1 : want > MAX_PARTS ? MAX_PARTS : want;
+  if (cus > 0 && N / (2 * cus) < S) S = N / (2 * cus);
+  if (S < 2) S = 1;
+  p.S = S;
+  int n0 = 0;
+  for (int i = 0; i < S; ++i) {
+    const int left = S - i, n = (N - n0 + left - 1) / left;
+    p.part[i] = Part{n0, n};
+    n0 += n;
+  }
+  return p;
+}
+
+inline size_t tile_floats(size_t tile_elems) { return 9 * tile_elems; }
+
+inline size_t p_region_off(const Part& pt, size_t tile_elems) { return (size_t)pt.n0 * tile_floats(tile_elems); }
+inline size_t p_region_floats(const Part& pt, size_t tile_elems) { return (size_t)pt.n * tile_floats(tile_elems); }
+
+struct FuseScratch { size_t edge_floats, nld; size_t floats() const { return edge_floats + 2 * nld + 4; } };
+inline FuseScratch fuse_scratch(size_t Q, size_t pxw) {
+  const size_t wgs = (Q + pxw - 1) / pxw;
+  return FuseScratch{(wgs * 4 * FUSE_EDGE_W * 4 + 3) & ~(size_t)3, wgs * (pxw / 32)};
+}
+inline bool fuse_scratch_fits(const FuseScratch& f, bool whole_call, size_t region_floats, size_t pstride) {
+  return f.floats() <= (whole_call ? 4 * pstride : region_floats);
+}
+
+}
diff --git a/audiosourcesep_amd/engine.py b/audiosourcesep_amd/engine.py
--- a/audiosourcesep_amd/engine.py
+++ b/audiosourcesep_amd/engine.py
@@ -195,6 +195,10 @@
     def fused_steps(self):
         return int(self.lib.glowk_fused_steps(self.h))
 
+    @property
+    def subbatch_calls(self):
+        return int(self.lib.glowk_subbatch_calls(self.h))
+
     def kernel_families(self):
         out = (ctypes.c_int64 * 7)()
         _lib.check(self.lib.glowk_kernel_families(self.h, out))
diff --git a/include/glowk.h b/include/glowk.h
--- a/include/glowk.h
+++ b/include/glowk.h
@@ -101,6 +101,7 @@
 } glowk_profile;
 int glowk_profile_begin(glowk_handle* h);
 int64_t glowk_fused_steps(const glowk_handle* h);
+int64_t glowk_subbatch_calls(const glowk_handle* h);
 int glowk_kernel_families(const glowk_handle* h, int64_t* out7);
 int glowk_profile_end(glowk_handle* h, glowk_profile* out);
 
```

Result: no change. 16990, median of 6 (+0.2%).
